# nzfeng/signed-heat-3d

Measured on AMD Instinct MI355X. Metric: grid-nodes/sec end-to-end SHM (conv+PCG), higher is better.
Workload: dtype f64 (Step 1: f64 / packed-f32 tiers)

## Files before the change

include/shm_grid.h:

```cpp
#ifndef SHM_GRID_H
#define SHM_GRID_H

#include <stddef.h>
#include <stdint.h>

#ifdef __cplusplus
extern "C" {
#endif

#define SHM_GRID_ABI_VERSION 5

typedef struct shm_solver shm_solver;

typedef enum {
    SHM_OK = 0,
    SHM_ERR_INVALID = 1,
    SHM_ERR_HIP = 2,
    SHM_ERR_NOMEM = 3,
    SHM_ERR_BREAKDOWN = 4,
    SHM_ERR_NOCONV = 5,
    SHM_ERR_RCCL = 6,
    SHM_ERR_STATE = 7,
    SHM_ERR_SINGULAR = 8
} shm_status;
// ... 24 lines not shown
    int32_t n;
    double bbox_min[3];
    double cell;
} shm_grid;

typedef struct {
    int32_t fast_integration;
    int32_t scrub_nonfinite;
    double tol;
    int32_t max_iters;
    int32_t check_every;
    int32_t preconditioner;
    int32_t solver;
    int32_t step1_arith;
    int32_t dual_form;
    double step1_budget;
} shm_opts;

enum { SHM_DUAL_AUTO = 0, SHM_DUAL_DIRECT = 1, SHM_DUAL_EXPLICIT_S_CG = 2, SHM_DUAL_THROUGH_GRID = 3 };

enum { SHM_STEP1_AUTO = 0, SHM_STEP1_EXACT_F64 = 1, SHM_STEP1_REFERENCE_F64 = 2 };

enum { SHM_SOLVER_AUTO = 0, SHM_SOLVER_PRIMAL = 1, SHM_SOLVER_DUAL = 2, SHM_SOLVER_DUAL_SLABS = 3 };

enum { SHM_PRECOND_AUTO = 0, SHM_PRECOND_NONE = 1, SHM_PRECOND_DCT = 2 };

typedef struct {
    int32_t n, m;
    int64_t S;
    int32_t iters;
    double rel_residual;
    double shift;
    double ms_conv;
    double ms_div;
    double ms_setup;
    double ms_wait_setup;
    double ms_pcg;
    double ms_shift;
    double ms_total;
    double ms_stencil_avg;
    double ms_update_xr_avg;
    double ms_project_avg;
    double ms_update_p_avg;
    double ms_precond_avg;
    int32_t kernel_samples;
    int32_t preconditioner;
    int32_t solver;
    double bytes_per_iter;
    int32_t cg_form;
    double pairs_fp64;
    double pairs_fp32;
    int32_t conv_launches;
    double pairs_redone;
} shm_stats;

shm_status shm_grid_create(const shm_config* cfg, shm_solver** out);
void shm_grid_destroy(shm_solver* s);
const char* shm_grid_last_error(const shm_solver* s);
int32_t shm_grid_abi_version(void);

shm_status shm_grid_set_problem(shm_solver* s, const shm_sources* src, const shm_grid* grid);
shm_status shm_grid_solve(shm_solver* s, const shm_opts* opts, shm_stats* stats);
shm_status shm_grid_get_phi(shm_solver* s, double* phi_out, int32_t* k_begin, int32_t* k_end);
shm_status shm_grid_owned_planes(shm_solver* s, int32_t* k_begin, int32_t* k_end);
shm_status shm_grid_compute_distance(shm_solver* s, const shm_sources* src, const shm_grid* grid,
                                     const shm_opts* opts, double* phi_out, shm_stats* stats);

typedef enum {
    SHM_FIELD_Y0 = 0,
    SHM_FIELD_Y1 = 1,
    SHM_FIELD_Y2 = 2,
    SHM_FIELD_DIV = 3,
    SHM_FIELD_PHI = 4
} shm_field;
shm_status shm_grid_run_conv(shm_solver* s);
shm_status shm_grid_run_conv_arith(shm_solver* s, int32_t step1_arith);
shm_status shm_grid_run_divergence(shm_solver* s, int32_t scrub);
shm_status shm_grid_get_field(shm_solver* s, shm_field f, double* out );
shm_status shm_grid_get_field_planes(shm_solver* s, shm_field f, int32_t k_begin, int32_t k_end, double* out);
shm_status shm_grid_apply_laplacian(shm_solver* s, const double* u, double* out);
shm_status shm_grid_set_phi(shm_solver* s, const double* phi );
shm_status shm_grid_get_constraints(shm_solver* s, int64_t* nodes, double* coeffs, int32_t* m);
shm_status shm_grid_get_schur(shm_solver* s, double* out, int32_t* m);
shm_status shm_grid_apply_projector(shm_solver* s, double* v);

shm_status shm_grid_apply_preconditioner(shm_solver* s, const double* v, double* out);

enum { SHM_ISO_MARCHING_CUBES = 0, SHM_ISO_MARCHING_TETS = 1 };
shm_status shm_grid_isosurface(shm_solver* s, double isovalue, int64_t* n_vertices, int64_t* n_triangles);
shm_status shm_grid_isosurface_ex(shm_solver* s, double isovalue, int32_t method, int64_t* n_vertices, int64_t* n_triangles);
shm_status shm_grid_get_isosurface(shm_solver* s, double* vertices , int64_t* triangles );

shm_status shm_grid_sample(shm_solver* s, int64_t Q, const double* pts, double* phi_out, double* grad_out, int64_t* n_answered);
shm_status shm_grid_sample_device(shm_solver* s, int64_t Q, const void* d_pts, void* d_phi, void* d_grad, int64_t* n_answered);

shm_status shm_grid_isosurface_indexed(shm_solver* s, double isovalue, int64_t* n_vertices, int64_t* n_triangles);
shm_status shm_grid_get_isosurface_indexed(shm_solver* s, double* vertices , int64_t* triangles );
shm_status shm_grid_get_isosurface_indexed_device(shm_solver* s, void* d_vertices , void* d_triangles );

typedef struct {
    int64_t first_vertex;
    int64_t n_vertices, n_triangles;
    double  area, volume;
    double  lo[3], hi[3];
    int32_t touches_box;
    int32_t reserved;
} shm_iso_component;
shm_status shm_grid_label_mesh_device(shm_solver* s, int64_t nv, int64_t nt, const void* d_triangles , void* d_root , int64_t* n_components);
shm_status shm_grid_isosurface_components(shm_solver* s, int64_t* n_components);
shm_status shm_grid_get_isosurface_components(shm_solver* s, shm_iso_component* comps , int64_t* tri_component ,
                                              int64_t* vertex_component );
shm_status shm_grid_isosurface_keep_components(shm_solver* s, const uint8_t* keep , int64_t* n_vertices, int64_t* n_triangles);

typedef struct {
    int64_t n_audited, n_not_owned, n_nonfinite, n_out_of_zone, n_finite_mismatch;
    double  max_dy;
    int64_t worst_node;
    double  worst_ratio;
    double  min_ratio;
    double  budget;
    int32_t step1_arith;
    int32_t within_budget;
    double  ms;
} shm_step1_audit;
shm_status shm_grid_audit_step1(shm_solver* s, int64_t count, const int64_t* nodes, double* dy_out , double* ratio_out ,
                                shm_step1_audit* out);
int64_t shm_audit_sample_nodes(int32_t n, int32_t k_begin, int32_t k_end, int64_t count, uint64_t seed, int64_t* nodes_out);

shm_status shm_grid_raycast(shm_solver* s, int64_t Q, const double* origins , const double* dirs , double isovalue, double t_min, double t_max,
                            double* t_out , double* grad_out , int64_t* n_hits);
shm_status shm_grid_raycast_device(shm_solver* s, int64_t Q, const void* d_origins, const void* d_dirs, double isovalue, double t_min, double t_max, void* d_t,
                                   void* d_grad, int64_t* n_hits);

typedef struct {
    int64_t n_frozen;
    int64_t n_reached;
    int64_t n_nonfinite;
    int64_t n_block_updates;
    int32_t n_rounds;
    int32_t reserved;
    double max_abs;
    double isovalue, band;
    double ms;
} shm_redistance_stats;
shm_status shm_grid_redistance(shm_solver* s, double isovalue, double band, shm_redistance_stats* out );
shm_status shm_grid_get_redistanced(shm_solver* s, double* psi_out );
shm_status shm_grid_get_redistanced_device(shm_solver* s, void* d_psi );

typedef struct {
    int64_t n_vertices, n_triangles;
    int64_t n_reached;
    int64_t n_candidate_pairs;
    double max_abs;
    double isovalue, band;
    double ms;
} shm_redistance_exact_stats;
shm_status shm_grid_redistance_exact(shm_solver* s, double isovalue, double band, shm_redistance_exact_stats* out );
shm_status shm_grid_isosurface_indexed_psi(shm_solver* s, double distance, int64_t* n_vertices, int64_t* n_triangles);

shm_status shm_grid_closest_point(shm_solver* s, int64_t Q, const double* pts , double max_dist, double* dist_out ,
                                  double* cp_out , int64_t* tri_out , int64_t* n_answered);
shm_status shm_grid_closest_point_device(shm_solver* s, int64_t Q, const void* d_pts, double max_dist, void* d_dist, void* d_cp ,
                                         void* d_tri , int64_t* n_answered);

shm_status shm_comm_unique_id(void* out128);
void shm_plan_slab(int32_t n, int32_t nslabs, int32_t slab, int32_t* k0, int32_t* k1);
// ... 8 lines not shown
```

signed-heat-3d_amd/csrc/shm_grid.hip:

```cpp
#include "shm_host.hip.h"
#include "shm_audit_sample.h"


struct shm_solver {
    std::unique_ptr<shm::SolverBase> impl;
    std::string err;
    shm_config cfg;
};

static thread_local std::string g_create_error;

template <typename F> static shm_status guard(shm_solver* s, F&& f) {
    if (!s) return SHM_ERR_INVALID;
    try {
        f();
        s->err.clear();
        return SHM_OK;
    } catch (const shm::Error& e) {
        s->err = e.what();
        return e.code;
    } catch (const std::bad_alloc&) {
        s->err = "host allocation failed";
        return SHM_ERR_NOMEM;
    } catch (const std::exception& e) {
// ... 82 lines not shown
    return guard(s, [&] {
        if (!src || !grid) throw shm::Error(SHM_ERR_INVALID, "null argument");
        s->impl->set_problem(*src, *grid);
    });
}

shm_status shm_grid_solve(shm_solver* s, const shm_opts* opts, shm_stats* stats) {
    return guard(s, [&] {
        shm_opts o;
        memset(&o, 0, sizeof o);
        o.scrub_nonfinite = 1;
        if (opts) o = *opts;
        s->impl->solve(o, stats);
    });
}

shm_status shm_grid_get_phi(shm_solver* s, double* phi_out, int32_t* k_begin, int32_t* k_end) {
    return guard(s, [&] {
        if (!phi_out) throw shm::Error(SHM_ERR_INVALID, "null phi_out");
        s->impl->get_phi(phi_out, k_begin, k_end);
    });
}

shm_status shm_grid_owned_planes(shm_solver* s, int32_t* k_begin, int32_t* k_end) {
    return guard(s, [&] { s->impl->owned_planes(k_begin, k_end); });
}

shm_status shm_grid_compute_distance(shm_solver* s, const shm_sources* src, const shm_grid* grid, const shm_opts* opts, double* phi_out,
                                     shm_stats* stats) {
    shm_status rc = shm_grid_set_problem(s, src, grid);
    if (rc != SHM_OK) return rc;
    if (s->cfg.world != 1) {
        s->err = "shm_grid_compute_distance is the single-process entry point; use set_problem/solve/get_phi per rank";
        return SHM_ERR_INVALID;
    }
    rc = shm_grid_solve(s, opts, stats);
    if (rc != SHM_OK && rc != SHM_ERR_NOCONV) return rc;
    std::string keep = s->err;
    shm_status rc2 = shm_grid_get_phi(s, phi_out, nullptr, nullptr);
    if (rc2 != SHM_OK) return rc2;
    s->err = keep;
    return rc;
}

shm_status shm_grid_run_conv(shm_solver* s) { return guard(s, [&] { s->impl->run_conv(SHM_STEP1_AUTO); }); }
shm_status shm_grid_run_conv_arith(shm_solver* s, int32_t step1_arith) { return guard(s, [&] { s->impl->run_conv(step1_arith); }); }
shm_status shm_grid_run_divergence(shm_solver* s, int32_t scrub) { return guard(s, [&] { s->impl->run_divergence(scrub); }); }
shm_status shm_grid_get_field(shm_solver* s, shm_field f, double* out) {
    return guard(s, [&] {
        if (!out) throw shm::Error(SHM_ERR_INVALID, "null out");
        s->impl->get_field(f, out);
    });
}
shm_status shm_grid_get_field_planes(shm_solver* s, shm_field f, int32_t k_begin, int32_t k_end, double* out) {
    return guard(s, [&] {
        if (!out) throw shm::Error(SHM_ERR_INVALID, "null out");
        s->impl->get_field_planes(f, k_begin, k_end, out);
    });
}
shm_status shm_grid_apply_laplacian(shm_solver* s, const double* u, double* out) {
    return guard(s, [&] {
        if (!u || !out) throw shm::Error(SHM_ERR_INVALID, "null argument");
        s->impl->apply_laplacian(u, out);
    });
}
shm_status shm_grid_set_phi(shm_solver* s, const double* phi) {
    return guard(s, [&] {
        if (!phi) throw shm::Error(SHM_ERR_INVALID, "null argument");
        s->impl->set_phi(phi);
    });
}
shm_status shm_grid_get_constraints(shm_solver* s, int64_t* nodes, double* coeffs, int32_t* m) {
    return guard(s, [&] {
        if (!nodes || !coeffs || !m) throw shm::Error(SHM_ERR_INVALID, "null argument");
        s->impl->get_constraints(nodes, coeffs, m);
    });
}
shm_status shm_grid_get_schur(shm_solver* s, double* out, int32_t* m) {
    return guard(s, [&] {
        if (!out || !m) throw shm::Error(SHM_ERR_INVALID, "null argument");
        s->impl->get_schur(out, m);
    });
}
shm_status shm_grid_apply_projector(shm_solver* s, double* v) {
    return guard(s, [&] {
        if (!v) throw shm::Error(SHM_ERR_INVALID, "null argument");
        s->impl->apply_projector(v);
    });
}

shm_status shm_grid_apply_preconditioner(shm_solver* s, const double* v, double* out) {
    return guard(s, [&] {
        if (!v || !out) throw shm::Error(SHM_ERR_INVALID, "null argument");
        s->impl->apply_preconditioner(v, out);
    });
}

shm_status shm_grid_isosurface(shm_solver* s, double isovalue, int64_t* n_vertices, int64_t* n_triangles) {
    return guard(s, [&] { s->impl->isosurface(isovalue, SHM_ISO_MARCHING_CUBES, n_vertices, n_triangles); });
}
shm_status shm_grid_isosurface_ex(shm_solver* s, double isovalue, int32_t method, int64_t* n_vertices, int64_t* n_triangles) {
    return guard(s, [&] { s->impl->isosurface(isovalue, method, n_vertices, n_triangles); });
}
shm_status shm_grid_get_isosurface(shm_solver* s, double* vertices, int64_t* triangles) {
    return guard(s, [&] { s->impl->get_isosurface(vertices, triangles); });
}

shm_status shm_grid_isosurface_indexed(shm_solver* s, double isovalue, int64_t* n_vertices, int64_t* n_triangles) {
    return guard(s, [&] { s->impl->isosurface_indexed(isovalue, n_vertices, n_triangles); });
}
shm_status shm_grid_get_isosurface_indexed(shm_solver* s, double* vertices, int64_t* triangles) {
    return guard(s, [&] { s->impl->get_isosurface_indexed(vertices, triangles); });
}
shm_status shm_grid_get_isosurface_indexed_device(shm_solver* s, void* d_vertices, void* d_triangles) {
    return guard(s, [&] { s->impl->get_isosurface_indexed_device(d_vertices, d_triangles); });
}

shm_status shm_grid_label_mesh_device(shm_solver* s, int64_t nv, int64_t nt, const void* d_triangles, void* d_root, int64_t* n_components) {
    return guard(s, [&] { s->impl->label_mesh_device(nv, nt, d_triangles, d_root, n_components); });
}
shm_status shm_grid_isosurface_components(shm_solver* s, int64_t* n_components) {
    return guard(s, [&] { s->impl->isosurface_components(n_components); });
}
shm_status shm_grid_get_isosurface_components(shm_solver* s, shm_iso_component* comps, int64_t* tri_component, int64_t* vertex_component) {
    return guard(s, [&] { s->impl->get_isosurface_components(comps, tri_component, vertex_component); });
}
shm_status shm_grid_isosurface_keep_components(shm_solver* s, const uint8_t* keep, int64_t* n_vertices, int64_t* n_triangles) {
    return guard(s, [&] { s->impl->isosurface_keep_components(keep, n_vertices, n_triangles); });
}

shm_status shm_grid_sample(shm_solver* s, int64_t Q, const double* pts, double* phi_out, double* grad_out, int64_t* n_answered) {
    return guard(s, [&] { s->impl->sample(Q, pts, phi_out, grad_out, n_answered); });
}
shm_status shm_grid_sample_device(shm_solver* s, int64_t Q, const void* d_pts, void* d_phi, void* d_grad, int64_t* n_answered) {
    return guard(s, [&] { s->impl->sample_device(Q, d_pts, d_phi, d_grad, n_answered); });
}

shm_status shm_grid_raycast(shm_solver* s, int64_t Q, const double* origins, const double* dirs, double isovalue, double t_min, double t_max, double* t_out,
                            double* grad_out, int64_t* n_hits) {
    return guard(s, [&] { s->impl->raycast(Q, origins, dirs, isovalue, t_min, t_max, t_out, grad_out, n_hits); });
}
shm_status shm_grid_raycast_device(shm_solver* s, int64_t Q, const void* d_origins, const void* d_dirs, double isovalue, double t_min, double t_max, void* d_t,
                                   void* d_grad, int64_t* n_hits) {
    return guard(s, [&] { s->impl->raycast_device(Q, d_origins, d_dirs, isovalue, t_min, t_max, d_t, d_grad, n_hits); });
}

shm_status shm_grid_redistance(shm_solver* s, double isovalue, double band, shm_redistance_stats* out) {
    return guard(s, [&] { s->impl->redistance(isovalue, band, out); });
}
shm_status shm_grid_redistance_exact(shm_solver* s, double isovalue, double band, shm_redistance_exact_stats* out) {
    return guard(s, [&] { s->impl->redistance_exact(isovalue, band, out); });
}
shm_status shm_grid_isosurface_indexed_psi(shm_solver* s, double distance, int64_t* n_vertices, int64_t* n_triangles) {
    return guard(s, [&] { s->impl->isosurface_indexed_psi(distance, n_vertices, n_triangles); });
}
shm_status shm_grid_get_redistanced(shm_solver* s, double* psi_out) {
    return guard(s, [&] { s->impl->get_redistanced(psi_out); });
}
shm_status shm_grid_get_redistanced_device(shm_solver* s, void* d_psi) {
    return guard(s, [&] { s->impl->get_redistanced_device(d_psi); });
}

shm_status shm_grid_closest_point(shm_solver* s, int64_t Q, const double* pts, double max_dist, double* dist_out, double* cp_out, int64_t* tri_out, int64_t* n_answered) {
    return guard(s, [&] { s->impl->closest_point(Q, pts, max_dist, dist_out, cp_out, tri_out, n_answered); });
}
shm_status shm_grid_closest_point_device(shm_solver* s, int64_t Q, const void* d_pts, double max_dist, void* d_dist, void* d_cp, void* d_tri, int64_t* n_answered) {
// ... 30 lines not shown
```

signed-heat-3d_amd/csrc/shm_host.hip.h:

```cpp
#pragma once
#include <hip/hip_runtime.h>
#include <rccl/rccl.h>

#include <dlfcn.h>

#include <algorithm>
#include <atomic>
#include <chrono>
#include <cmath>
#include <cstdarg>
#include <cstdio>
#include <cstring>
#include <limits>
#include <memory>
#include <mutex>
#include <stdexcept>
#include <string>
#include <thread>
#include <unordered_map>
#include <unordered_set>
#include <vector>

#include "../../include/shm_grid.h"
#include "shm_constraints.h"
// ... 409 lines not shown
                            lbs[(size_t)(s - g0)] = rel - lhs_drop;
                            if (lbs[(size_t)(s - g0)] <= ln_tau) {
                                bnd[(size_t)(s - g0)] = std::exp(lbs[(size_t)(s - g0)]) * r_hi / d_box;
                                gsum += bnd[(size_t)(s - g0)];
                            }
                        }
                        const bool soft_ok = R + gsum <= eps_soft;
                        if (soft_ok) R += gsum;
                        for (int64_t s = g0; s < g1; s++) {
                            if (!(wmag[(size_t)s] > 0.)) continue;
                            if (bnd[(size_t)(s - g0)] >= 0. && (soft_ok || lbs[(size_t)(s - g0)] <= ln_tau_hard)) continue;
                            const double lhs = lambda * (dist[(size_t)s] - rt - r_hi), rel = std::log(wmag[(size_t)s]) - ln_near;
                            const double d_box = std::max(0., dist[(size_t)s] - rt), d0 = std::max(0., dmin - rt);
                            const bool in_range = 1.4426950408889634 * lambda * (d_box - d0) + range_c <= std::log2(wmag[(size_t)s]) - lwhi;
                            cost += lhs > tier_log + rel && in_range ? far_cost : 1.0;
                        }
                    }
                } else {
                    for (size_t c = 0; c < crad.size(); c++) {
                        const double dx = cx - ccen[3 * c], dy = cy - ccen[3 * c + 1], dz = cz - ccen[3 * c + 2];
                        const double gap = std::sqrt(dx * dx + dy * dy + dz * dz) - rt - crad[c] - r_hi;
                        if (!(gap * lambda > skip_base + clnw[c] - ln_near)) cost += kCl;
                    }
                }
                acc += cost;
            }
        const double per_plane = acc / ((double)K * K * (double)S) + 1e-3;
        for (int k = L * bz; k < std::min(n, (L + 1) * bz); k++) weights[k] = per_plane;
    };
    const unsigned hw = std::thread::hardware_concurrency();
    const int nthr = (int)std::max(1u, std::min({hw ? hw : 1u, 16u, (unsigned)layers, (unsigned)(((double)layers * K * K * (double)S) / 2e6 + 1.)}));
    std::atomic<int> next{0};
    auto worker = [&]() {
        std::vector<double> dist((size_t)S);
        for (int L = next.fetch_add(1); L < layers; L = next.fetch_add(1)) do_layer(L, dist);
    };
    std::vector<std::thread> pool;
    for (int t = 1; t < nthr; t++) pool.emplace_back(worker);
    worker();
    for (std::thread& t : pool) t.join();
}

static void plan_slabs_weighted(int n, int nslabs, const double* w, int granule, std::vector<int32_t>& bounds) {
    bounds.assign((size_t)nslabs + 1, 0);
    bounds[(size_t)nslabs] = n;
    if (granule < 1) granule = 1;
    if ((long long)granule * nslabs > n) granule = std::max(1, n / nslabs);
    std::vector<double> cum((size_t)n + 1, 0.);
    for (int k = 0; k < n; k++) cum[(size_t)k + 1] = cum[(size_t)k] + (w && w[k] > 0. ? w[k] : 0.);
    if (!(cum[(size_t)n] > 0.))
        for (int k = 0; k <= n; k++) cum[(size_t)k] = k;
    for (int i = 1; i < nslabs; i++) {
        const double target = cum[(size_t)n] * i / nslabs;
        const int lo = bounds[(size_t)i - 1] + granule, hi = n - (nslabs - i) * granule;
        int best = lo;
        double best_err = 1e300;
        for (int k = ((lo + granule - 1) / granule) * granule; k <= hi; k += granule) {
            const double e = std::fabs(cum[(size_t)k] - target);
            if (e < best_err) {
                best_err = e;
                best = k;
            }
        }
        bounds[(size_t)i] = std::min(std::max(best, lo), std::max(lo, hi));
    }
}

struct SolverBase {
    virtual ~SolverBase() = default;
    virtual void set_problem(const shm_sources&, const shm_grid&) = 0;
    virtual void solve(const shm_opts&, shm_stats*) = 0;
    virtual void get_phi(double*, int32_t*, int32_t*) = 0;
    virtual void owned_planes(int32_t*, int32_t*) = 0;
    virtual void run_conv(int step1_arith) = 0;
    virtual void run_divergence(int scrub) = 0;
    virtual void get_field(shm_field, double*) = 0;
    virtual void get_field_planes(shm_field, int, int, double*) = 0;
    virtual void apply_laplacian(const double*, double*) = 0;
    virtual void set_phi(const double*) = 0;
    virtual void get_constraints(int64_t*, double*, int32_t*) = 0;
    virtual void apply_projector(double*) = 0;
    virtual void apply_preconditioner(const double*, double*) = 0;
    virtual void get_schur(double*, int32_t*) = 0;
    virtual void isosurface(double, int, int64_t*, int64_t*) = 0;
    virtual void get_isosurface(double*, int64_t*) = 0;
    virtual void sample(int64_t, const double*, double*, double*, int64_t*) = 0;
    virtual void sample_device(int64_t, const void*, void*, void*, int64_t*) = 0;
    virtual void isosurface_indexed(double, int64_t*, int64_t*) = 0;
    virtual void get_isosurface_indexed(double*, int64_t*) = 0;
    virtual void get_isosurface_indexed_device(void*, void*) = 0;
    virtual void label_mesh_device(int64_t, int64_t, const void*, void*, int64_t*) = 0;
    virtual void isosurface_components(int64_t*) = 0;
    virtual void get_isosurface_components(shm_iso_component*, int64_t*, int64_t*) = 0;
    virtual void isosurface_keep_components(const uint8_t*, int64_t*, int64_t*) = 0;
    virtual void audit_step1(int64_t, const int64_t*, double*, double*, shm_step1_audit*) = 0;
    virtual void raycast(int64_t, const double*, const double*, double, double, double, double*, double*, int64_t*) = 0;
    virtual void raycast_device(int64_t, const void*, const void*, double, double, double, void*, void*, int64_t*) = 0;
    virtual void redistance(double, double, shm_redistance_stats*) = 0;
    virtual void get_redistanced(double*) = 0;
    virtual void get_redistanced_device(void*) = 0;
    virtual void redistance_exact(double, double, shm_redistance_exact_stats*) = 0;
    virtual void isosurface_indexed_psi(double, int64_t*, int64_t*) = 0;
    virtual void closest_point(int64_t, const double*, double, double*, double*, int64_t*, int64_t*) = 0;
    virtual void closest_point_device(int64_t, const void*, double, void*, void*, void*, int64_t*) = 0;
};

SolverBase* make_solver_f64(const shm_config& cfg);
SolverBase* make_solver_f32(const shm_config& cfg);

}
```

signed-heat-3d_amd/csrc/shm_kernels.hip.h:

```cpp
#pragma once
#include <hip/hip_runtime.h>
#include <stdint.h>

#include <type_traits>

#include "shm_constraints.h"
#include "shm_mc_table.h"

namespace shm {

constexpr int kBlock = 256;
constexpr int kMaxPartials = 8192;

__device__ __forceinline__ double wave_sum(double v) {
#pragma unroll
    for (int off = 32; off > 0; off >>= 1) v += __shfl_down(v, off, kWave);
    return v;
}

__device__ __forceinline__ double block_sum(double v, double* lds ) {
    v = wave_sum(v);
    const int lane = threadIdx.x & 63, w = threadIdx.x >> 6;
    if (lane == 0) lds[w] = v;
    __syncthreads();
    double s = 0.;
    if (threadIdx.x == 0) {
        const int nw = (blockDim.x * blockDim.y + 63) >> 6;
        for (int a = 0; a < nw; a++) s += lds[a];
    }
    return s;
}

__device__ __forceinline__ unsigned xcd_remap(unsigned bid, unsigned nblk) {
    const unsigned xcd = bid & 7u, slot = bid >> 3;
    const unsigned q = nblk >> 3, r = nblk & 7u;
    const unsigned base = (xcd < r) ? xcd * (q + 1) : r * (q + 1) + (xcd - r) * q;
    return base + slot;
}

constexpr int kSrcTile = 256;

template <typename T> struct YukawaMath;
template <> struct YukawaMath<double> {
    static constexpr int kExpTabBits = 11;
    static __device__ __forceinline__ double yukawa(double x, double c, const double* __restrict__ tab ) {
        const double y0 = __builtin_amdgcn_rsq(x);
        const double t = x * y0;
        const double e = fma(-t, y0, 1.0);
        const double q = fma(e, 0.375, 0.5) * e;
        const double r = fma(t, q, t);
        const double rinv = fma(y0, q, y0);
        const double tm = fma(r, c, 6755399441055744.0);
        const double kf = tm - 6755399441055744.0;
        const int ki = (int)(unsigned)__double_as_longlong(tm);
        const double f = fma(r, c, -kf);
        double p = 6.461528672932366e-12;
        p = fma(p, f, 5.727446245172041e-08);
        p = fma(p, f, 3.384507717577858e-04);
        p = fma(p, f, 1.0);
        return __builtin_amdgcn_ldexp(tab[ki & ((1 << kExpTabBits) - 1)] * p * rinv, ki >> kExpTabBits);
    }
    static __device__ __forceinline__ double exp_neg(double x) {
        const double kf = rint(x * 1.4426950408889634074);
        double f = fma(kf, -6.93147180369123816490e-01, x);
        f = fma(kf, -1.90821492927058770002e-10, f);
        double p = 1.6059043836821613e-10;
        p = fma(p, f, 2.08767569878681e-09);
        p = fma(p, f, 2.505210838544172e-08);
        p = fma(p, f, 2.755731922398589e-07);
        p = fma(p, f, 2.7557319223985893e-06);
        p = fma(p, f, 2.48015873015873e-05);
        p = fma(p, f, 1.984126984126984e-04);
        p = fma(p, f, 1.3888888888888889e-03);
        p = fma(p, f, 8.333333333333333e-03);
        p = fma(p, f, 4.1666666666666664e-02);
        p = fma(p, f, 1.6666666666666666e-01);
        p = fma(p, f, 0.5);
        p = fma(p, f, 1.0);
        p = fma(p, f, 1.0);
        return __builtin_amdgcn_ldexp(p, (int)kf);
    }
};
template <> struct YukawaMath<float> {
    static __device__ __forceinline__ void rsqrt_and_sqrt(float x, float& rinv, float& r) {
        const float y0 = __builtin_amdgcn_rsqf(x);
        r = x * y0;
        rinv = y0;
    }
    static __device__ __forceinline__ float exp_neg(float x) { return __expf(x); }
// ... 1394 lines not shown
            const int j = t & (kGJ - 1), k2 = t >> 6;
            rs[k2][j] = R[(size_t)(r_row0 + kc + k2) * ld + oj + j];
        }
        __syncthreads();
#pragma unroll
        for (int kk = 0; kk < kGJK; kk += 4) {
            double af[2], bf[2];
#pragma unroll
            for (int a = 0; a < 2; a++) af[a] = cs[wr * 32 + a * 16 + l15][kk + l4];
#pragma unroll
            for (int b = 0; b < 2; b++) bf[b] = rs[kk + l4][wc * 32 + b * 16 + l15];
#pragma unroll
            for (int a = 0; a < 2; a++)
#pragma unroll
                for (int b = 0; b < 2; b++) acc[a][b] = __builtin_amdgcn_mfma_f64_16x16x4f64(af[a], bf[b], acc[a][b], 0, 0, 0);
        }
    }
    const bool prow = kb >= 0 && bi == kb, pcol = kb >= 0 && bj == kb;
    const size_t o = (size_t)kb * kGJ;
#pragma unroll
    for (int a = 0; a < 2; a++)
#pragma unroll
        for (int b = 0; b < 2; b++)
#pragma unroll
            for (int r = 0; r < 4; r++) {
                const size_t row = oi + wr * 32 + a * 16 + l4 + 4 * r, col = oj + wc * 32 + b * 16 + l15;
                double* dst = &G[row * ld + col];
                const double v = acc[a][b][r];
                if (prow) *dst = R[(size_t)(r_row0 + (int)(row - o)) * ld + col];
                else if (pcol) *dst = -v;
                else *dst -= v;
            }
}
template <int TILES>
__global__ __launch_bounds__(kBlock) void gj_update_kernel(double* __restrict__ G_, int ld, int nb, int kb ,
                                                           int k0, int nO, const double* __restrict__ R_ , int r_row0,
                                                           const double* __restrict__ C_ , int c_ld, int c_col0, int K, int prio,
                                                           GjBatch Bt = GjBatch{nullptr, nullptr, nullptr, nullptr, nullptr, nullptr, nullptr}) {
    __shared__ double smem[kGjUpdateLds];
    if (prio) __builtin_amdgcn_s_setprio(3);
    double* G = G_;
    const double* R = R_;
    const double* C = C_;
    if (Bt.D) {
        const int a = blockIdx.y;
        ld = gj_batch_ld(Bt, a);
        nb = ld / kGJ;
        if (kb >= nb || blockIdx.x >= (unsigned)(nb * (nb + 1) / 2)) return;
        G = Bt.D + Bt.offD[a];
        R = Bt.R + Bt.offW[a];
        C = Bt.C + Bt.offW[a];
        c_ld = kGJ;
    }
    int bi, bj;
    if (TILES == GJ_ALL) {
        gj_tri_decode(blockIdx.x, bi, bj);
    } else if (TILES == GJ_CROSS) {
        const int idx = (int)blockIdx.x;
        if (idx < nO * nb) {
            bj = k0 + idx % nO;
            bi = idx / nO;
            if (bi < bj) return;
        } else {
            const int r = idx - nO * nb;
            bi = k0 + r % nO;
            bj = r / nO;
        }
    } else {
        gj_tri_decode(blockIdx.x, bi, bj);
        if (bi >= k0) bi += nO;
        if (bj >= k0) bj += nO;
    }
    gj_update_tile(G, ld, bi, bj, TILES != GJ_REST ? kb : -1, R, r_row0, C, c_ld, c_col0, K, smem);
}

#ifndef SHM_GJ_STEP_PAIRS
#define SHM_GJ_STEP_PAIRS 1
#endif
#ifndef SHM_GJ_STEP_WAVES
#define SHM_GJ_STEP_WAVES 3
#endif
constexpr int kGjStepScratch = 8 * (kGJ + 1);
constexpr int kGjStepLds = kGJ * (kGJ + 1) + kGjStepScratch;
static __global__ __launch_bounds__(kBlock) __attribute__((amdgpu_waves_per_eu(SHM_GJ_STEP_WAVES, SHM_GJ_STEP_WAVES))) void gj_step_kernel(
    double* __restrict__ G, int ld, int nb, int k, const double* __restrict__ Rp , const double* __restrict__ Cp ,
    double* __restrict__ Rn, double* __restrict__ Cn, int* __restrict__ flag, int prio) {
    __shared__ double smem[kGjStepLds];
    static_assert(kGjStepLds >= kGjUpdateLds && kGjStepScratch >= 8 * kGJ, "LDS carve");
    if (prio) __builtin_amdgcn_s_setprio(3);
    const int nN = k < nb ? nb : 0;
    if ((int)blockIdx.x >= nN) {
        int bi, bj;
        gj_tri_decode(blockIdx.x - (unsigned)nN, bi, bj);
        if (k < nb) {
            if (bi >= k) bi += 1;
            if (bj >= k) bj += 1;
        }
        gj_update_tile(G, ld, bi, bj, k - 1, Rp, 0, Cp, kGJ, 0, kGJ, smem);
        return;
    }
    double(*x)[kGJ + 1] = reinterpret_cast<double(*)[kGJ + 1]>(smem);
    double* scratch = smem + kGJ * (kGJ + 1);
    double(*prow)[kGJ + 1] = reinterpret_cast<double(*)[kGJ + 1]>(scratch);
    const int b = blockIdx.x;
    const bool below = b >= k;
    const int bi = below ? b : k, bj = below ? k : b;
    const size_t o = (size_t)k * kGJ, ob = (size_t)b * kGJ, oi = (size_t)bi * kGJ, oj = (size_t)bj * kGJ;
    const int lane = threadIdx.x & 63, w = threadIdx.x >> 6, wr = w >> 1, wc = w & 1, l15 = lane & 15, l4 = lane >> 4;
    const int ty = threadIdx.x >> 4, tx = threadIdx.x & 15;
    double r[4][4];
    double* Cb = Cn + ob * kGJ;
    if (k > 0) {
        auto product = [&](gj_f64x4(&acc)[2][2], size_t orow, size_t ocol) {
#pragma unroll
            for (int a = 0; a < 2; a++)
#pragma unroll
                for (int c = 0; c < 2; c++) acc[a][c] = gj_f64x4{0., 0., 0., 0.};
#pragma unroll 1
            for (int g = 0; g < 2; g++) {
                double af[8][2], bf[8][2];
#pragma unroll
                for (int u = 0; u < 8; u++) {
                    const int kk = 32 * g + 4 * u + l4;
#pragma unroll
                    for (int a = 0; a < 2; a++) af[u][a] = Cp[(orow + wr * 32 + a * 16 + l15) * kGJ + kk];
#pragma unroll
                    for (int c = 0; c < 2; c++) bf[u][c] = Rp[(size_t)kk * ld + ocol + wc * 32 + c * 16 + l15];
                }
#pragma unroll
                for (int u = 0; u < 8; u++)
#pragma unroll
                    for (int a = 0; a < 2; a++)
#pragma unroll
                        for (int c = 0; c < 2; c++) acc[a][c] = __builtin_amdgcn_mfma_f64_16x16x4f64(af[u][a], bf[u][c], acc[a][c], 0, 0, 0);
            }
        };
        {
            gj_f64x4 accp[2][2];
            product(accp, o, o);
#pragma unroll
            for (int a = 0; a < 2; a++)
#pragma unroll
                for (int c = 0; c < 2; c++)
#pragma unroll
                    for (int q = 0; q < 4; q++) {
                        const size_t row = wr * 32 + a * 16 + l4 + 4 * q, col = wc * 32 + c * 16 + l15;
                        x[row][col] = G[(o + row) * ld + o + col] - accp[a][c][q];
                    }
        }
        gj_f64x4 accx[2][2];
        product(accx, oi, oj);
        __syncthreads();
#pragma unroll
        for (int a = 0; a < 4; a++)
#pragma unroll
            for (int c = 0; c < 4; c++) r[a][c] = x[ty * 4 + a][tx * 4 + c];
        __syncthreads();
        const double keep = b == k - 1 ? 0. : 1.;
#pragma unroll
        for (int a = 0; a < 2; a++)
#pragma unroll
            for (int c = 0; c < 2; c++)
#pragma unroll
                for (int q = 0; q < 4; q++) {
                    const size_t row = wr * 32 + a * 16 + l4 + 4 * q, col = wc * 32 + c * 16 + l15;
                    x[row][col] = G[(oi + row) * ld + oj + col] * keep - accx[a][c][q];
                }
    } else {
        for (int t = threadIdx.x; t < kGJ * kGJ; t += kBlock) {
            const int i = t / kGJ, j = t % kGJ;
            x[i][j] = G[(oi + i) * ld + oj + j];
        }
#pragma unroll
        for (int a = 0; a < 4; a++)
#pragma unroll
            for (int c = 0; c < 4; c++) r[a][c] = G[(o + ty * 4 + a) * ld + o + tx * 4 + c];
    }
    __syncthreads();
    for (int t = threadIdx.x; t < kGJ * kGJ; t += kBlock) {
        const int i = t / kGJ, j = t % kGJ;
        Cb[i * kGJ + j] = below ? x[i][j] : -x[j][i];
    }
    gj_invert64_scalar<4, SHM_GJ_STEP_PAIRS != 0>(r, scratch, flag);
    if (b == k) {
#pragma unroll
        for (int a = 0; a < 4; a++)
#pragma unroll
            for (int c = 0; c < 4; c++) Rn[(size_t)(ty * 4 + a) * ld + ob + tx * 4 + c] = r[a][c];
        return;
    }
    double pa[2][kGJ / 4];
#pragma unroll
    for (int pass = 0; pass < 8; pass++) {
        __syncthreads();
        if ((ty >> 1) == pass) {
#pragma unroll
            for (int a = 0; a < 4; a++)
#pragma unroll
                for (int c = 0; c < 4; c++) prow[(ty & 1) * 4 + a][tx * 4 + c] = r[a][c];
        }
        __syncthreads();
        if (wr == (pass >> 2) && (l15 >> 3) == (pass & 1)) {
#pragma unroll
            for (int s4 = 0; s4 < kGJ / 4; s4++) pa[(pass >> 1) & 1][s4] = prow[l15 & 7][4 * s4 + l4];
        }
    }
    gj_f64x4 acc[2][2];
#pragma unroll
    for (int a = 0; a < 2; a++)
#pragma unroll
        for (int c = 0; c < 2; c++) acc[a][c] = gj_f64x4{0., 0., 0., 0.};
#pragma unroll
    for (int s4 = 0; s4 < kGJ / 4; s4++) {
        const int kk = 4 * s4 + l4;
        double bf[2];
#pragma unroll
        for (int c = 0; c < 2; c++) {
            const int j = wc * 32 + c * 16 + l15;
            bf[c] = (b > k) ? x[j][kk] : x[kk][j];
        }
#pragma unroll
        for (int a = 0; a < 2; a++)
#pragma unroll
            for (int c = 0; c < 2; c++) acc[a][c] = __builtin_amdgcn_mfma_f64_16x16x4f64(pa[a][s4], bf[c], acc[a][c], 0, 0, 0);
    }
#pragma unroll
    for (int a = 0; a < 2; a++)
#pragma unroll
        for (int c = 0; c < 2; c++)
#pragma unroll
            for (int q = 0; q < 4; q++) Rn[(size_t)(wr * 32 + a * 16 + l4 + 4 * q) * ld + ob + wc * 32 + c * 16 + l15] = acc[a][c][q];
}

static __global__ __launch_bounds__(kBlock) void gj_mirror_kernel(double* __restrict__ G_, int ld, GjBatch Bt = GjBatch{nullptr, nullptr, nullptr, nullptr, nullptr, nullptr, nullptr}) {
    __shared__ double x[kGJ][kGJ + 1];
    double* G = G_;
    if (Bt.D) {
        const int a = blockIdx.y;
        ld = gj_batch_ld(Bt, a);
        const int nb = ld / kGJ;
        if (blockIdx.x >= (unsigned)(nb * (nb - 1) / 2)) return;
        G = Bt.D + Bt.offD[a];
    }
    const unsigned t = blockIdx.x;
    int bi = (int)((sqrt(8.0 * (double)t + 1.0) - 1.0) * 0.5);
    while ((unsigned)bi * (unsigned)(bi + 1) / 2 > t) bi--;
    while ((unsigned)(bi + 1) * (unsigned)(bi + 2) / 2 <= t) bi++;
    const int bj = (int)(t - (unsigned)bi * (unsigned)(bi + 1) / 2);
    bi += 1;
    const size_t oi = (size_t)bi * kGJ, oj = (size_t)bj * kGJ;
    for (int e = threadIdx.x; e < kGJ * kGJ; e += kBlock) {
        const int i = e / kGJ, j = e % kGJ;
        x[i][j] = G[(oi + i) * ld + oj + j];
    }
    __syncthreads();
    for (int e = threadIdx.x; e < kGJ * kGJ; e += kBlock) {
        const int i = e / kGJ, j = e % kGJ;
        G[(oj + i) * ld + oi + j] = x[j][i];
    }
}

struct IsoParams {
    int n, nzl, k0;
    double bbox_min[3];
    double cell;
    double iso;
};

__device__ __constant__ int kKuhnTets[6][4] = {{0, 1, 3, 7}, {0, 1, 5, 7}, {0, 2, 3, 7}, {0, 2, 6, 7}, {0, 4, 5, 7}, {0, 4, 6, 7}};

__device__ __forceinline__ int tet_tris(int mask) {
    const int c = __popc(mask);
    return c == 0 || c == 4 ? 0 : (c == 2 ? 2 : 1);
}

template <typename T, bool EMIT>
__global__ __launch_bounds__(kBlock) void iso_kernel(IsoParams P, const T* __restrict__ phi , unsigned long long* __restrict__ counter,
                                                     double* __restrict__ tri_pos , unsigned long long* __restrict__ tri_keys ,
                                                     unsigned long long* __restrict__ tri_sort , unsigned long long cap) {
    __shared__ double red[8];
    const int n = P.n, nc = n - 1;
    const size_t plane = (size_t)n * n;
    const int kend = min(P.nzl, n - 1 - P.k0);
    const size_t ncells = (size_t)nc * nc * (size_t)max(kend, 0);
    double mycount = 0.;
    for (size_t c = (size_t)blockIdx.x * kBlock + threadIdx.x; c < ncells; c += (size_t)gridDim.x * kBlock) {
        const int kk = (int)(c / ((size_t)nc * nc));
        const int rem = (int)(c - (size_t)kk * nc * nc);
        const int j = rem / nc, i = rem - j * nc;
        const size_t base = (size_t)(kk + 1) * plane + (size_t)j * n + i;
        double v[8];
        int inside = 0;
        bool fin = true;
#pragma unroll
        for (int q = 0; q < 8; q++) {
            v[q] = (double)phi[base + (q & 1) + ((q >> 1) & 1) * (size_t)n + ((q >> 2) & 1) * plane];
            inside |= (v[q] < P.iso ? 1 : 0) << q;
            fin &= v[q] - v[q] == 0.;
        }
        if (inside == 0 || inside == 255 || !fin) continue;
        const int k = P.k0 + kk;
        const unsigned long long gnode = (unsigned long long)i + (unsigned long long)j * n + (unsigned long long)k * plane;
        for (int t = 0; t < 6; t++) {
            int tv[4], mask = 0;
#pragma unroll
            for (int a = 0; a < 4; a++) {
                tv[a] = kKuhnTets[t][a];
                mask |= ((inside >> tv[a]) & 1) << a;
            }
            const int nt = tet_tris(mask);
            if (nt == 0) continue;
            if (!EMIT) {
                mycount += nt;
                continue;
// ... 128 lines not shown
```

signed-heat-3d_amd/csrc/shm_plan.h:

```cpp
#pragma once
#include <algorithm>
#include <cmath>
#include <cstdint>
#include <cstdlib>

#include "../../include/shm_grid.h"

namespace shm {

enum Step1Kernel { kStep1TieredF64, kStep1TieredF32, kStep1Untiered };
enum PlanPath { kPathFast, kPathGathered, kPathDualSlabs, kPathDualLocal, kPathPrimalFused, kPathPrimalClassic };

struct PlanKnobs {
    bool no_direct = false;
    bool no_dense_s = false;
    bool dense_s_always = false;
    int tl_min_m = 6144;
};
template <typename Get> PlanKnobs plan_knobs(Get knob) {
    PlanKnobs k;
    k.no_direct = knob("SHM_DUAL_NO_DIRECT") != nullptr;
    k.no_dense_s = knob("SHM_DUAL_NO_DENSE_S") != nullptr;
    k.dense_s_always = knob("SHM_DUAL_DENSE_S_ALWAYS") != nullptr;
    if (knob("SHM_TL_MIN_M")) k.tl_min_m = atoi(knob("SHM_TL_MIN_M"));
    return k;
}

struct PlanIn {
    bool f64 = true;
    int n = 0;
    int64_t S = 0;
    int total_slabs = 1;
    bool full_wanted = false, fft_available = false, gemm_dct = false, fused_available = false;
    Step1Kernel step1 = kStep1Untiered;
    double conv_est_total_ms = 1e30;
    int solver = SHM_SOLVER_AUTO, preconditioner = SHM_PRECOND_AUTO, dual_form = SHM_DUAL_AUTO;
    double step1_budget = 0.;
    bool fast = false;
    PlanKnobs knobs;
    bool precond_available() const { return fft_available || gemm_dct; }
    bool tiered() const { return step1 != kStep1Untiered; }
};

struct Plan {
    shm_status status = SHM_OK;
    const char* error = nullptr;
    PlanPath path = kPathPrimalClassic;
    bool precond = false;
    bool dual_requested = false;
    int setup_prio = 1;
    bool green_early = false;
    int dual_form = SHM_DUAL_THROUGH_GRID;
    bool explicit_S = false;
    bool two_level = false;
    double est_setup_ms = -1., est_step1_ms = -1.;
};

inline Plan plan_error(shm_status s, const char* msg) { Plan p; p.status = s; p.error = msg; return p; }

inline Plan plan_solve(const PlanIn& in) {
    Plan p;
    if (in.preconditioner == SHM_PRECOND_DCT) {
        if (!in.precond_available())
            return plan_error(SHM_ERR_INVALID, "DCT preconditioner needs n = 2^k in [16,1024] and a power-of-two number of EQUAL z-slabs dividing n (shm_config.slab_plan = SHM_SLAB_PLAN_EQUAL); a single z-slab serves any n in [4,1024]");
        p.precond = true;
    } else if (in.preconditioner == SHM_PRECOND_AUTO) {
        p.precond = in.precond_available();
    } else if (in.preconditioner != SHM_PRECOND_NONE) {
        return plan_error(SHM_ERR_INVALID, "unknown preconditioner");
    }
    if (in.dual_form < SHM_DUAL_AUTO || in.dual_form > SHM_DUAL_THROUGH_GRID) return plan_error(SHM_ERR_INVALID, "unknown dual_form");
    if (in.step1_budget != 0. && !(in.step1_budget >= 1e-12 && in.step1_budget <= 1e-3)) return plan_error(SHM_ERR_INVALID, "step1_budget must lie in [1e-12, 1e-3] (0: default 1e-8)");
    if (in.solver != SHM_SOLVER_AUTO && in.solver != SHM_SOLVER_PRIMAL && in.solver != SHM_SOLVER_DUAL && in.solver != SHM_SOLVER_DUAL_SLABS)
        return plan_error(SHM_ERR_INVALID, "unknown solver");
    if (in.fast) {
        p.path = kPathFast;
        return p;
    }
    const bool with_precond = in.preconditioner != SHM_PRECOND_NONE;
    const bool slab_forms_auto = in.solver == SHM_SOLVER_AUTO && with_precond && in.fft_available && in.total_slabs >= 4 && in.n >= 256 && in.n <= 512 && in.S <= 16384 &&
                                 in.dual_form != SHM_DUAL_THROUGH_GRID;
    if (in.full_wanted && !slab_forms_auto && (in.solver == SHM_SOLVER_AUTO || in.solver == SHM_SOLVER_DUAL) && with_precond) {
        p.path = kPathGathered;
        return p;
    }
    p.dual_requested = (in.solver == SHM_SOLVER_DUAL || in.solver == SHM_SOLVER_DUAL_SLABS || (in.solver == SHM_SOLVER_AUTO && with_precond)) && in.precond_available();
    bool dual = false;
    if (in.solver == SHM_SOLVER_DUAL || in.solver == SHM_SOLVER_DUAL_SLABS) {
        if (!in.precond_available())
            return plan_error(SHM_ERR_INVALID, "the dual solver needs the DCT: n = 2^k in [16,1024] and a power-of-two number of EQUAL z-slabs dividing n (shm_config.slab_plan = SHM_SLAB_PLAN_EQUAL); a single z-slab serves any n in [4,1024]");
        dual = true;
    } else if (in.solver == SHM_SOLVER_AUTO) {
        dual = in.precond_available() && with_precond;
    }
    if (dual) p.path = in.total_slabs > 1 ? kPathDualSlabs : kPathDualLocal;
    else p.path = in.fused_available ? kPathPrimalFused : kPathPrimalClassic;
    return p;
}

inline void plan_setup(const PlanIn& in, Plan& p) {
    p.setup_prio = in.step1 == kStep1TieredF64 && in.conv_est_total_ms >= 150. && in.conv_est_total_ms < 1e29 ? 0 : 1;
    const bool iterative_form = in.dual_form == SHM_DUAL_EXPLICIT_S_CG || in.dual_form == SHM_DUAL_THROUGH_GRID;
    p.green_early = !iterative_form && p.dual_requested && !in.knobs.no_direct && !in.knobs.no_dense_s && (in.total_slabs == 1 || in.fft_available) &&
                    in.precond_available() && !in.gemm_dct && in.n <= 512 && in.S > 0 && in.S <= 4096 &&
                    (in.f64 || in.step1 == kStep1TieredF32 || in.n < 512 || in.dual_form == SHM_DUAL_DIRECT);
}

inline bool plan_explicit_S(const PlanIn& in, int m, bool direct) {
    const bool off = in.knobs.no_dense_s || in.dual_form == SHM_DUAL_THROUGH_GRID;
    if (in.gemm_dct) return !off && m > 0 && m <= 16384;
    if (in.total_slabs > 1) return !off && in.fft_available && m > 0 && m <= 16384 && in.n <= 512;
    const bool asked = in.dual_form == SHM_DUAL_DIRECT || in.dual_form == SHM_DUAL_EXPLICIT_S_CG;
    const int max_m = (in.tiered() || asked) ? 16384 : 8192;
    if (off || !in.precond_available() || m <= 0 || m > max_m || in.n > 512) return false;
    if (in.knobs.dense_s_always || asked || direct) return true;
    const double md = (double)m, width = in.f64 ? 1.0 : 0.5;
    const double schur_est_ms = 2.2e-7 * md * md;
    const double dense_iter_ms = 3.6e-9 * md * md * width + 0.08;
    const double grid_iter_ms = std::max(0.15, 1.4 * std::pow((double)in.n / 512.0, 3.0) * width);
    return in.tiered() && in.conv_est_total_ms >= 3.0 * schur_est_ms && grid_iter_ms > 1.3 * dense_iter_ms;
}

template <typename Est> void plan_rows(const PlanIn& in, int m, Est step1_ms, Plan& p) {
    const bool no_direct = in.knobs.no_direct || in.dual_form == SHM_DUAL_EXPLICIT_S_CG || in.dual_form == SHM_DUAL_THROUGH_GRID;
    const int direct_max_m = in.dual_form == SHM_DUAL_DIRECT ? 16384 : 4096;
    bool direct = p.dual_requested && !no_direct && m <= direct_max_m;
    if (!direct && p.dual_requested && !no_direct && in.tiered() && in.precond_available() && !in.gemm_dct && in.n <= 512 && m > direct_max_m && m <= 16384 &&
        in.conv_est_total_ms < 1e29) {
        const double md = (double)m;
        p.est_setup_ms = 5.5e-11 * md * md * md + 1.4e-7 * md * md + 10.0 * std::pow((double)in.n / 512.0, 4.0);
        p.est_step1_ms = step1_ms();
        direct = p.est_setup_ms <= 0.38 * p.est_step1_ms;
    }
    if (!in.f64 && in.step1 != kStep1TieredF32 && in.n >= 512 && !in.gemm_dct && in.dual_form != SHM_DUAL_DIRECT) direct = false;
    direct = direct && plan_explicit_S(in, m, true);
    p.explicit_S = plan_explicit_S(in, m, direct);
    p.dual_form = direct ? SHM_DUAL_DIRECT : p.explicit_S ? SHM_DUAL_EXPLICIT_S_CG : SHM_DUAL_THROUGH_GRID;
    p.two_level = !direct && m > in.knobs.tl_min_m;
}

inline const char* plan_path_name(PlanPath path) {
    static const char* const names[] = {"fast", "gathered", "dual-slabs", "dual", "primal-fused", "primal-classic"};
    return names[path];
}

}
```

signed-heat-3d_amd/csrc/shm_solver.hip.h:

```cpp
#pragma once
#include "shm_host.hip.h"
#include "shm_kernels.hip.h"
#include "shm_conv_tiered.hip.h"
#include "shm_cg_fused.hip.h"
#include "shm_twolevel.hip.h"
#include "shm_schur.hip.h"
#include "shm_dct.hip.h"
#include "shm_dct_gemm.hip.h"
#include "shm_green_fft.hip.h"
#include "shm_sample.hip.h"
#include "shm_audit.hip.h"
#include "shm_iso_indexed.hip.h"
#include "shm_iso_components.hip.h"
#include "shm_raycast.hip.h"
#include "shm_redistance.hip.h"
#include "shm_redistance_exact.hip.h"
#include "shm_closest.hip.h"
#include "shm_plan.h"

namespace shm {

template <typename T> constexpr int vec_width() { return sizeof(T) == 8 ? 2 : 4; }

template <typename T>
// ... 44 lines not shown
    double conv_ctr[3] = {0, 0, 0};
    double conv_wscale = 1.;
    int64_t S = 0;
    std::vector<double> h_pos, h_wn, h_area;
    double area_sum = 0., conv_far_gap = 0., conv_skip_base = 3.0e38, last_host_setup_ms = 0., last_setup_wall_ms = 0.;
    double conv_tier_ring = 0.;
    double conv_tier_log = 0., conv_tier_skip_base = 3.0e38;
    double conv_drop_K = 64., conv_drop_eps64 = 2e-9, conv_drop_eps32 = 6.0e-8;
    double conv_w_span = 0.;
    DevArray<double> d_src_t;
    DevArray<float> d_clusters_t;
    int n_clusters_t = 0;
    bool conv_tiered = false;
    bool conv_tier_exact = false;
    bool conv_tiered32 = false;
    bool conv_reference = false;
    int step1_selected = SHM_STEP1_AUTO;
    int last_step1_arith = SHM_STEP1_AUTO;
    double last_step1_budget = 0.;
    bool fold_pq = false;
    int fold_pq_np = 0;
    double step1_budget = 0.;
    DevArray<unsigned long long> d_pair_counters;
    DevArray<unsigned> d_unit_counters;
    static constexpr int kMaxConvLaunches = 256;
    int conv_launch_index = 0;
    int conv_launches_last = 0;
    int n_clusters = 0;
    int conv_grid_cap = 1 << 30;
    bool o_fast_hint = false;
    int num_cus = 256;
    DevArray<T> d_src;
    DevArray<float> d_src32;
    DevArray<float> d_clusters;
    DevArray<double> d_exptab;
    std::vector<Slab<T>> slabs;
    int total_slabs = 1, first_slab = 0;
    std::vector<int32_t> slab_bounds;
    bool slabs_equal = true;
    void slab_range(int slab, int32_t* k0, int32_t* k1) const {
        *k0 = slab_bounds[(size_t)slab];
        *k1 = slab_bounds[(size_t)slab + 1];
    }
    bool have_problem = false, have_conv = false, have_div = false, have_phi = false, have_constraints = false;
    std::vector<Row> rows;
    std::vector<std::vector<ShiftItem>> shift_host;
    int m = 0, mp = 0;
    DevArray<double> Ginv, gjP, gjR, gjC;
    DevArray<float> Ginv32;
    struct TwoLevel {
        bool on = false;
        int box = 16, P = 0, nI = 0, nS = 0, nSp = 0, ysz = 0;
        DevArray<int> ptrI, ptrS, rowsI, colsS, sepRow, adj_ptr, adj_idx, colour_list, rowBox, chunkBox, chunkCol, tBox, tRow, sBox, sRow;
        DevArray<size_t> offW;
        DevArray<double> gjP, gjR, gjC;
        int nChunks = 0, nTChunks = 0, nbMax = 0;
        int schur_ptr[9] = {0, 0, 0, 0, 0, 0, 0, 0, 0};
        DevArray<size_t> offD, offE;
        DevArray<double> D, E, Tm, tbuf, ybuf, vS, uS;
        DevArray<float> D32, E32, T32;
        int colour_ptr[9] = {0, 0, 0, 0, 0, 0, 0, 0, 0};
        size_t szD = 0, szE = 0;
        TlBoxes view() const { return TlBoxes{ptrI.p, ptrS.p, offD.p, offE.p, rowsI.p, colsS.p}; }
    } tl;
    int ginv_rows = 0, ginv_ld = 0;
    DevArray<int> gjFlag;
    DevArray<double*> d_redptrs;
    DevArray<int> Bptr, Bcol;
    DevArray<double> Bval;
    bool have_B = false;
    using TP = T;
    DevArray<Cplx<TP>> d_tw, d_om;
    DevArray<TP> d_lam;
    DevArray<double> d_lam64;
    DevArray<double> gd_Cm, gd_Ct, gd_W1, gd_W2;
    DevArray<double> gs_lam, gs_ctab, gs_Cm, gs_Ct, gs_W0, gs_W1, gs_T, Sdense, d_rowT;
    DevArray<int> d_rowX;
    std::vector<double> h_gs_lam, h_gs_ctab, h_rowT;
    std::vector<Cplx<double>> h_gs_tw;
    DevArray<Cplx<double>> gs_tw;
    std::vector<int> h_rowX;
    bool have_S = false;
    DevArray<double> Sinv, Sinv_ones ;
    PlanIn plan_in;
    Plan plan;
    double conv_est_total_ms = 1e30;
    int log2n = 0;
    bool precond_ready = false;
    double* h_pinned = nullptr;
    Rccl::comm_t comm = nullptr;
    int vec = 1;
    std::unique_ptr<Solver<T>> full;
    bool solve_only = false;
    bool full_problem_set = false;
    bool pool_held = false;

    explicit Solver(const shm_config& c, bool solve_only_ = false) : cfg(c), solve_only(solve_only_) {
        int ndev = 0;
        hipError_t e = hipGetDeviceCount(&ndev);
        if (e != hipSuccess || ndev <= 0)
            throw Error(SHM_ERR_HIP, fmt("no HIP device available (%s); this library has no CPU fallback",
                                          e == hipSuccess ? "device count 0" : hipGetErrorString(e)));
        if (cfg.device < 0 || cfg.device >= ndev) throw Error(SHM_ERR_INVALID, fmt("device %d out of range [0,%d)", cfg.device, ndev));
        HIPCHK(hipSetDevice(cfg.device));
        HIPCHK(hipStreamCreateWithFlags(&stream, hipStreamNonBlocking));
        {
            hipDeviceProp_t prop;
            HIPCHK(hipGetDeviceProperties(&prop, cfg.device));
            conv_grid_cap = std::max(1, prop.multiProcessorCount * 4);
            num_cus = prop.multiProcessorCount;
        }
        {
            int least = 0, greatest = 0;
            HIPCHK(hipDeviceGetStreamPriorityRange(&least, &greatest));
            HIPCHK(hipStreamCreateWithPriority(&stream2, hipStreamNonBlocking, greatest));
        }
        HIPCHK(hipHostMalloc((void**)&h_pinned, 64 * sizeof(double)));
        if (cfg.world > 1 && !cfg.rccl_unique_id) throw Error(SHM_ERR_INVALID, "world>1 needs rccl_unique_id");
        if (cfg.rccl_unique_id) {
            Rccl& R = Rccl::get();
            Rccl::unique_id id;
            memcpy(&id, cfg.rccl_unique_id, sizeof id);
            R.chk(R.CommInitRank(&comm, cfg.world, id, cfg.rank), "ncclCommInitRank");
        }
        PinnedPool::get().acquire(cfg.device);
        pool_held = true;
    }
    ~Solver() override {
        (void)hipSetDevice(cfg.device);
        if (comm) (void)Rccl::get().CommDestroy(comm);
        if (h_pinned) (void)hipHostFree(h_pinned);
        for (void* b : smp_pinned)
            if (b) (void)hipHostFree(b);
        for (void* b : ray_pinned)
            if (b) (void)hipHostFree(b);
        slabs.clear();
        if (stream) (void)hipStreamDestroy(stream);
        if (stream2) (void)hipStreamDestroy(stream2);
        if (stream3) (void)hipStreamDestroy(stream3);
        if (stream_h) (void)hipStreamDestroy(stream_h);
        if (pool_held) PinnedPool::get().release(cfg.device);
    }

    void log(const char* f, ...) {
        if (!cfg.verbose) return;
        va_list ap;
        va_start(ap, f);
        vfprintf(stderr, f, ap);
        va_end(ap);
        fputc('\n', stderr);
    }

    static int grid_for(size_t work_items, int cap = 2048) {
        size_t b = (work_items + kBlock - 1) / kBlock;
        if (b < 1) b = 1;
        if (b > (size_t)cap) b = cap;
        return (int)b;
    }

    void set_problem(const shm_sources& src, const shm_grid& g) override {
        HIPCHK(hipSetDevice(cfg.device));
        if (g.n < 2) throw Error(SHM_ERR_INVALID, "grid.n must be >= 2");
        if (!(g.cell > 0.) || !std::isfinite(g.cell)) throw Error(SHM_ERR_INVALID, "grid.cell must be positive and finite");
        if (src.S <= 0 || !src.pos || !src.wnormal || !src.area) throw Error(SHM_ERR_INVALID, "sources: S>0 and non-null arrays required");
        if (!(src.lambda > 0.) || !std::isfinite(src.lambda)) throw Error(SHM_ERR_INVALID, "sources.lambda must be positive and finite");
        if (src.S > (int64_t)1 << 28) throw Error(SHM_ERR_INVALID, "too many sources");
// ... 889 lines not shown
        HIPCHK(hipGetLastError());
        log("[shm] two-level inverse of A A^T: box %d, %d boxes (%d interior rows, largest box %d rows x %d separator columns), separator %d rows", tl.box, P, tl.nI, part.maxs, part.maxc, tl.nS);
        return true;
    }

    void apply_Ginv(const double* w, double* u, bool f32, hipStream_t st) {
        if (m <= 0) return;
        if (!tl.on) {
            if (f32) launch_ginv_matvec<float>(st, m, m, mp, Ginv32.p, w, u);
            else launch_ginv_matvec<double>(st, m, m, mp, Ginv.p, w, u);
            return;
        }
        const TlBoxes V = tl.view();
        const unsigned grows = (unsigned)((tl.nI + kBlock / kWave - 1) / (kBlock / kWave));
        if (f32) hipLaunchKernelGGL((tl_rows_kernel<float>), dim3(grows), dim3(kBlock), 0, st, V, tl.rowBox.p, tl.nI, tl.D32.p, w, tl.tbuf.p);
        else hipLaunchKernelGGL((tl_rows_kernel<double>), dim3(grows), dim3(kBlock), 0, st, V, tl.rowBox.p, tl.nI, tl.D.p, w, tl.tbuf.p);
        if (tl.nChunks > 0) {
            if (f32) hipLaunchKernelGGL((tl_cols_kernel<float>), dim3((unsigned)tl.nChunks), dim3(kBlock), 0, st, V, tl.chunkBox.p, tl.chunkCol.p, tl.E32.p, tl.tbuf.p, tl.ybuf.p);
            else hipLaunchKernelGGL((tl_cols_kernel<double>), dim3((unsigned)tl.nChunks), dim3(kBlock), 0, st, V, tl.chunkBox.p, tl.chunkCol.p, tl.E.p, tl.tbuf.p, tl.ybuf.p);
        }
        hipLaunchKernelGGL(tl_gather_sep_kernel, dim3((unsigned)((tl.nS + kBlock - 1) / kBlock)), dim3(kBlock), 0, st, tl.nS, tl.sepRow.p, tl.adj_ptr.p, tl.adj_idx.p, w,
                           tl.ybuf.p, tl.vS.p);
        if (f32) launch_ginv_matvec<float>(st, tl.nS, tl.nS, tl.nSp, Ginv32.p, tl.vS.p, tl.uS.p);
        else launch_ginv_matvec<double>(st, tl.nS, tl.nS, tl.nSp, Ginv.p, tl.vS.p, tl.uS.p);
        const unsigned gfin = grows + (unsigned)((tl.nS + kBlock - 1) / kBlock);
        if (f32) hipLaunchKernelGGL((tl_finish_kernel<float>), dim3(gfin), dim3(kBlock), 0, st, V, tl.rowBox.p, tl.nI, tl.nS, tl.sepRow.p, tl.T32.p, tl.tbuf.p, tl.uS.p, u);
        else hipLaunchKernelGGL((tl_finish_kernel<double>), dim3(gfin), dim3(kBlock), 0, st, V, tl.rowBox.p, tl.nI, tl.nS, tl.sepRow.p, tl.Tm.p, tl.tbuf.p, tl.uS.p, u);
    }

    void enqueue_gj_invert(double* M, int mp, bool refined_later = false) {
        hipStream_t stream = stream2;
        const int nb = mp / kGJ;
        const int outer = nb >= 64 ? 4 : 1;
        gjP.alloc(kGJ * kGJ);
        gjR.alloc((size_t)outer * kGJ * mp);
        gjC.alloc((size_t)mp * outer * kGJ);
        gjFlag.alloc(2);
        HIPCHK(hipMemsetAsync(gjFlag.p, 0, sizeof(int), stream));
        const int c_ld = outer * kGJ;
        const bool classic = knob("SHM_GJ_CLASSIC") != nullptr;
        const bool stepped = outer == 1 && !classic;
        auto launch_pivot = [&](int kb) {
            if (refined_later) hipLaunchKernelGGL(gj_pivot_block4_kernel, dim3(1), dim3(256), 0, stream, M, mp, kb, gjP.p, gjFlag.p, plan.setup_prio);
            else hipLaunchKernelGGL(gj_pivot_kernel<4>, dim3(1), dim3(256), 0, stream, M, mp, kb, gjP.p, gjFlag.p, plan.setup_prio);
        };
        if (stepped) {
            gjR.alloc((size_t)2 * kGJ * mp);
            gjC.alloc((size_t)2 * mp * kGJ);
            for (int k = 0; k <= nb; k++) {
                const size_t nU = k == 0 ? 0 : (k < nb ? (size_t)(nb - 1) * nb / 2 : (size_t)nb * (nb + 1) / 2);
                const unsigned grid = (unsigned)((k < nb ? nb : 0) + nU);
                double* Rn = gjR.p + (size_t)(k & 1) * kGJ * mp;
                double* Cn = gjC.p + (size_t)(k & 1) * mp * kGJ;
                const double* Rp = gjR.p + (size_t)((k + 1) & 1) * kGJ * mp;
                const double* Cp = gjC.p + (size_t)((k + 1) & 1) * mp * kGJ;
                hipLaunchKernelGGL(gj_step_kernel, dim3(grid), dim3(kBlock), 0, stream, M, mp, nb, k, Rp, Cp, Rn, Cn, gjFlag.p, plan.setup_prio);
            }
        } else if (outer == 1) {
            for (int kb = 0; kb < nb; kb++) {
                launch_pivot(kb);
                hipLaunchKernelGGL(gj_panels_kernel, dim3(nb), dim3(kBlock), 0, stream, M, mp, kb, gjP.p, gjR.p, 0, gjC.p, c_ld, 0, plan.setup_prio);
                hipLaunchKernelGGL((gj_update_kernel<GJ_ALL>), dim3((unsigned)((size_t)nb * (nb + 1) / 2)), dim3(kBlock), 0, stream, M, mp, nb, kb, 0, 1,
                                   gjR.p, 0, gjC.p, c_ld, 0, kGJ, plan.setup_prio);
            }
        } else {
            for (int k0 = 0; k0 < nb; k0 += outer) {
                const int nO = std::min(outer, nb - k0);
                for (int t = 0; t < nO; t++) {
                    const int kb = k0 + t;
                    launch_pivot(kb);
                    hipLaunchKernelGGL(gj_panels_kernel, dim3(nb), dim3(kBlock), 0, stream, M, mp, kb, gjP.p, gjR.p, t * kGJ, gjC.p, c_ld, t * kGJ, plan.setup_prio);
                    hipLaunchKernelGGL((gj_update_kernel<GJ_CROSS>), dim3((unsigned)(nO * nb + nO * k0)), dim3(kBlock), 0, stream, M, mp, nb, kb, k0, nO,
                                       gjR.p, t * kGJ, gjC.p, c_ld, t * kGJ, kGJ, plan.setup_prio);
                }
                const size_t nr = (size_t)(nb - nO);
                if (nr > 0)
                    hipLaunchKernelGGL((gj_update_kernel<GJ_REST>), dim3((unsigned)(nr * (nr + 1) / 2)), dim3(kBlock), 0, stream, M, mp, nb, -1, k0, nO,
                                       gjR.p, 0, gjC.p, c_ld, 0, nO * kGJ, plan.setup_prio);
            }
        }
        if (nb > 1) hipLaunchKernelGGL(gj_mirror_kernel, dim3((unsigned)((size_t)nb * (nb - 1) / 2)), dim3(kBlock), 0, stream, M, mp);
        HIPCHK(hipGetLastError());
    }
    void enqueue_invert_G() {
        const int mp = ginv_ld;
        enqueue_gj_invert(Ginv.p, mp);
        Ginv32.alloc((size_t)mp * mp);
        hipLaunchKernelGGL((convert_kernel<double, float>), dim3(grid_for((size_t)mp * mp, 4096)), dim3(kBlock), 0, stream2, (size_t)mp * mp, Ginv.p, Ginv32.p);
        HIPCHK(hipGetLastError());
    }
    void enqueue_green_table(hipStream_t st) {
        const int P = n + 8;
        const size_t n1 = (size_t)n + 1;
        {
            const double pi = 3.14159265358979323846;
            h_gs_lam.resize(n);
            h_gs_ctab.resize(2 * (size_t)n);
            for (int k = 0; k < n; k++) h_gs_lam[k] = (2. - 2. * std::cos(pi * k / n)) / (cell * cell);
            for (int r = 0; r < 2 * n; r++) h_gs_ctab[r] = std::cos(pi * r / n);
            gs_lam.upload(h_gs_lam, st);
            gs_ctab.upload(h_gs_ctab, st);
            gs_T.alloc(n1 * n1 * P);
        }
        {
            DevArray<double>&W0 = gs_W0, &W1 = gs_W1, &W2 = gs_W0;
            gs_Cm.alloc(n1 * n);
            gs_Ct.alloc((size_t)n * P);
            W0.alloc(std::max((size_t)n * n * n, (size_t)n * n1 * P));
            W1.alloc((size_t)n * n * P);
            const bool by_fft = (n & (n - 1)) == 0 && n >= 16 && n <= 512;
            if (by_fft) {
                const double pi = 3.14159265358979323846;
                h_gs_tw.resize(2 * (size_t)n);
                for (int t = 0; t < n; t++) {
                    h_gs_tw[(size_t)t] = {std::cos(2. * pi * t / n), -std::sin(2. * pi * t / n)};
                    h_gs_tw[(size_t)n + t] = {std::cos(pi * t / n), -std::sin(pi * t / n)};
                }
                gs_tw.upload(h_gs_tw, st);
                HIPCHK(hipMemsetAsync(W1.p, 0, (size_t)n * n * P * sizeof(double), st));
                hipLaunchKernelGGL(green_symbol_kernel, dim3((unsigned)std::min(n * n, 8 * num_cus)), dim3(kBlock), 0, st, n, gs_lam.p, W0.p);
                const long long Pl = P, n1l = (long long)n1;
                auto pass = [&](bool xpass, int ntiles, int tiles_a, DctAddr in, DctAddr out, const double* src, double* dst) {
                    CosiParams C;
                    C.ntiles = ntiles;
                    C.tiles_a = tiles_a;
                    C.in = in;
                    C.out = out;
                    const dim3 g((unsigned)std::min(ntiles, 16 * num_cus));
                    const Cplx<double>*tw = gs_tw.p, *om = gs_tw.p + n;
                    int l2 = 0;
                    while ((1 << l2) < n) l2++;
#define SHM_COSI_CASE(L)                                                                                                                              \
    case L:                                                                                                                                            \
        if (xpass) hipLaunchKernelGGL((cosi_lines_kernel<L, true>), g, dim3(kBlock), 0, st, C, src, dst, tw, om, plan.setup_prio);                         \
        else hipLaunchKernelGGL((cosi_lines_kernel<L, false>), g, dim3(kBlock), 0, st, C, src, dst, tw, om, plan.setup_prio);                              \
        break;
                    switch (l2) {
                        SHM_COSI_CASE(4) SHM_COSI_CASE(5) SHM_COSI_CASE(6) SHM_COSI_CASE(7) SHM_COSI_CASE(8) SHM_COSI_CASE(9)
                        default: throw Error(SHM_ERR_INVALID, "Green's table by FFT: n out of range");
                    }
#undef SHM_COSI_CASE
                };
                auto addr = [](long long a_stride, long long b_stride, long long line_stride, long long elem_stride) {
                    DctAddr A;
                    A.off = 0; A.a_stride = a_stride; A.b_stride = b_stride; A.line_stride = line_stride; A.elem_stride = elem_stride;
                    A.seg_stride = 0; A.seg_shift = 30; A.seg_mask = 0x3fffffff;
                    return A;
                };
                const int L = kCosiL;
                pass(true, n * n / L, n * n / L, addr((long long)L * n, 0, n, 1), addr((long long)L * Pl, 0, Pl, 1), W0.p, W1.p);
                pass(false, n * (P / L), P / L, addr(L, (long long)n * Pl, 1, Pl), addr(L, n1l * Pl, 1, Pl), W1.p, W2.p);
                pass(false, (int)(n1l * Pl / L), (int)(n1l * Pl / L), addr(L, 0, 1, n1l * Pl), addr(L, 0, 1, n1l * Pl), W2.p, gs_T.p);
                HIPCHK(hipGetLastError());
                return;
            }
            HIPCHK(hipMemsetAsync(gs_Ct.p, 0, (size_t)n * P * sizeof(double), st));
            hipLaunchKernelGGL(cosine_tables_kernel, dim3(grid_for(n1 * n, 1024)), dim3(kBlock), 0, st, n, P, gs_ctab.p, gs_Cm.p, gs_Ct.p);
            hipLaunchKernelGGL(green_symbol_kernel, dim3((unsigned)std::min(n * n, 8 * num_cus)), dim3(kBlock), 0, st, n, gs_lam.p, W0.p);
            const bool narrow = plan_in.tiered();
            auto tiles = [](size_t v) { return (unsigned)((v + kGemmT - 1) / kGemmT); };
            auto gemm = [&](unsigned batches, int M, int N, int K, const double* A, int lda, long long sA, const double* B, int ldb, long long sB, double* C, int ldc, long long sC) {
                if (narrow)
                    hipLaunchKernelGGL(dgemm_rm_kernel<1>, dim3((unsigned)((N + 31) / 32), tiles((size_t)M), batches), dim3(kBlock), 0, st, M, N, K, A, lda, sA, B, ldb, sB, C, ldc, sC, plan.setup_prio);
                else
                    hipLaunchKernelGGL(dgemm_rm_kernel<4>, dim3(tiles((size_t)N), tiles((size_t)M), batches), dim3(kBlock), 0, st, M, N, K, A, lda, sA, B, ldb, sB, C, ldc, sC, plan.setup_prio);
            };
            gemm(1, n * n, P, n, W0.p, n, 0LL, gs_Ct.p, P, 0LL, W1.p, P, 0LL);
            gemm((unsigned)n, (int)n1, P, n, gs_Cm.p, n, 0LL, W1.p, P, (long long)n * P, W2.p, P, (long long)(n1 * P));
            gemm(1, (int)n1, (int)(n1 * P), n, gs_Cm.p, n, 0LL, W2.p, (int)(n1 * P), 0LL, gs_T.p, (int)(n1 * P), 0LL);
            HIPCHK(hipGetLastError());
        }
    }
    void prepare_schur() {
        hipStream_t st = stream2;
        have_S = false;
        if (!plan.explicit_S) return;
        if (!plan.green_early) enqueue_green_table(st);
        schur_row_order(rows, h_rowX, h_rowT);
        d_rowX.upload(h_rowX, st);
        d_rowT.upload(h_rowT, st);
        Sdense.alloc((size_t)mp * mp);
        if (!stream3) {
            int least = 0, greatest = 0;
            HIPCHK(hipDeviceGetStreamPriorityRange(&least, &greatest));
            HIPCHK(hipStreamCreateWithPriority(&stream3, hipStreamNonBlocking, greatest));
            e_sch_in.reset(new Event());
            e_sch_done.reset(new Event());
        }
        e_sch_in->record(st);
    }
    void enqueue_schur() {
        if (!plan.explicit_S) return;
        const bool dual_direct = plan.dual_form == SHM_DUAL_DIRECT;
        hipStream_t st = dual_direct ? stream2 : stream3;
        HIPCHK(hipStreamWaitEvent(st, e_sch_in->e, 0));
        const int P = n + 8;
        if (plan.green_early) HIPCHK(hipStreamWaitEvent(st, e_gs_done->e, 0));
        HIPCHK(hipMemsetAsync(Sdense.p, 0, (size_t)mp * mp * sizeof(double), st));
        const unsigned mt = (unsigned)((m + 15) / 16);
        hipLaunchKernelGGL(schur_assemble_kernel, dim3(mt, mt), dim3(kBlock), 0, st, m, mp, n, P, d_rowX.p, d_rowT.p, gs_T.p, Sdense.p, plan.setup_prio);
        HIPCHK(hipGetLastError());
        if (dual_direct) {
            Sinv.alloc((size_t)mp * mp);
            HIPCHK(hipMemcpyAsync(Sinv.p, Sdense.p, (size_t)mp * mp * sizeof(double), hipMemcpyDeviceToDevice, st));
            if (mp > m) hipLaunchKernelGGL(set_diagonal_kernel, dim3((unsigned)((mp - m + kBlock - 1) / kBlock)), dim3(kBlock), 0, st, Sinv.p, mp, m, mp, 1.0);
            enqueue_gj_invert(Sinv.p, mp, true);
            Sinv_ones.alloc((size_t)2 * mp);
            hipLaunchKernelGGL(fill_kernel, dim3((unsigned)((m + kBlock - 1) / kBlock)), dim3(kBlock), 0, st, Sinv_ones.p + mp, m, 1.0);
            launch_ginv_matvec<double>(st, m, m, mp, Sinv.p, Sinv_ones.p + mp, Sinv_ones.p);
        } else {
            e_sch_done->record(st);
            HIPCHK(hipStreamWaitEvent(stream2, e_sch_done->e, 0));
        }
        have_S = true;
    }
    void finish_invert_G() {
        hipStream_t stream = stream2;
        int flag[2] = {0, 0};
        if (!tl.on) HIPCHK(hipMemsetAsync(gjFlag.p + 1, 0, sizeof(int), stream));
        HIPCHK(hipMemcpyAsync(flag, gjFlag.p, 2 * sizeof(int), hipMemcpyDeviceToHost, stream));
        HIPCHK(hipStreamSynchronize(stream));
        if (flag[0] || flag[1]) throw Error(SHM_ERR_SINGULAR, "A A^T is not positive definite (duplicate or degenerate constraint rows)");
    }

    void allreduce(int which , int count) {
        auto buf = [&](Slab<T>& sl) { return which == 0 ? sl.red.p : sl.pq.p; };
        if (slabs.size() > 1) {
            double** slot = d_redptrs.p + (which ? slabs.size() : 0);
            hipLaunchKernelGGL(sum_slabs_kernel, dim3((count + kBlock - 1) / kBlock), dim3(kBlock), 0, stream, (int)slabs.size(), slot, count);
        }
        if (comm) {
            Rccl& R = Rccl::get();
            R.chk(R.AllReduce(buf(slabs[0]), buf(slabs[0]), (size_t)count, Rccl::kFloat64, Rccl::kSum, comm, stream), "ncclAllReduce");
            for (size_t s = 1; s < slabs.size(); s++)
                HIPCHK(hipMemcpyAsync(buf(slabs[s]), buf(slabs[0]), (size_t)count * sizeof(double), hipMemcpyDeviceToDevice, stream));
        }
    }

    void halo_exchange_p() { halo_exchange(ARR_P); }
    void halo_exchange(int sel) { halo_exchange(sel, stream); }
    void halo_exchange(int sel, hipStream_t stream) {
        const size_t pb = slabs[0].plane * sizeof(T);
        for (size_t s = 0; s + 1 < slabs.size(); s++) {
            Slab<T>&a = slabs[s], &b = slabs[s + 1];
            HIPCHK(hipMemcpyAsync(arr(b, sel), arr(a, sel) + (size_t)a.nzl * a.plane, pb, hipMemcpyDeviceToDevice, stream));
            HIPCHK(hipMemcpyAsync(arr(a, sel) + (size_t)(a.nzl + 1) * a.plane, arr(b, sel) + b.plane, pb, hipMemcpyDeviceToDevice, stream));
        }
        if (comm) {
            Rccl& R = Rccl::get();
            const int dt = sizeof(T) == 8 ? Rccl::kFloat64 : Rccl::kFloat32;
            Slab<T>&lo = slabs.front(), &hi = slabs.back();
            const size_t cnt = lo.plane;
            R.chk(R.GroupStart(), "ncclGroupStart");
            if (cfg.rank > 0) {
                R.chk(R.Send(arr(lo, sel) + lo.plane, cnt, dt, cfg.rank - 1, comm, stream), "ncclSend(lo)");
                R.chk(R.Recv(arr(lo, sel), cnt, dt, cfg.rank - 1, comm, stream), "ncclRecv(lo)");
            }
            if (cfg.rank < cfg.world - 1) {
                R.chk(R.Send(arr(hi, sel) + (size_t)hi.nzl * hi.plane, cnt, dt, cfg.rank + 1, comm, stream), "ncclSend(hi)");
                R.chk(R.Recv(arr(hi, sel) + (size_t)(hi.nzl + 1) * hi.plane, cnt, dt, cfg.rank + 1, comm, stream), "ncclRecv(hi)");
            }
            R.chk(R.GroupEnd(), "ncclGroupEnd");
        }
    }

    struct StencilLaunch {
        dim3 grid, block;
        int xchunks, yblocks, zc;
    };
    StencilLaunch stencil_dims(const Slab<T>& sl) const {
        const int per_row = (n + vec - 1) / vec;
        int tx = 1;
        while (tx < per_row && tx < kBlock) tx <<= 1;
        const int tyb = kBlock / tx;
        const int xchunks = (per_row + tx - 1) / tx;
        const int yblocks = (n + tyb * kStRY - 1) / (tyb * kStRY);
        int zc = 16;
        while (zc > 4 && (long long)xchunks * yblocks * ((sl.nzl + zc - 1) / zc) < 1024) zc >>= 1;
        const int zchunks = (sl.nzl + zc - 1) / zc;
        return {dim3((unsigned)(xchunks * yblocks * zchunks)), dim3((unsigned)tx, (unsigned)tyb), xchunks, yblocks, zc};
    }

    void launch_stencil(Slab<T>& sl) {
        const StencilLaunch L = stencil_dims(sl);
        if (vec == 1)
            hipLaunchKernelGGL((stencil_dot_kernel<T, 1>), L.grid, L.block, 0, stream, sl.gp, L.xchunks, L.yblocks, L.zc, sl.p.p, sl.q.p, sl.partials.p);
        else
            hipLaunchKernelGGL((stencil_dot_kernel<T, vec_width<T>()>), L.grid, L.block, 0, stream, sl.gp, L.xchunks, L.yblocks, L.zc, sl.p.p, sl.q.p, sl.partials.p);
    }

    template <int VEC> void launch_update_xr(Slab<T>& sl, int rho_slot, int grid) {
        hipLaunchKernelGGL((update_xr_kernel<T, VEC>), dim3(grid), dim3(kBlock), 0, stream, sl.nown / VEC, sl.plane, sl.sc.p, rho_slot, sl.pq.p,
// ... 565 lines not shown
        enum { V_MU = 0, V_R = 1, V_P = 2, V_Z = 3, V_T1 = 4, V_T2 = 5, V_G = 6 };
        const std::vector<int> nopart(slabs.size(), 0);
        auto gather = [&](int sel) {
            for (Slab<T>& sl : slabs)
                hipLaunchKernelGGL((gather_rows_kernel<T>), dim3(1 + (8 * m + kBlock - 1) / kBlock), dim3(kBlock), 0, stream, m, sl.row_ptr.p, sl.ent_node.p,
                                   sl.ent_coef.p, arr(sl, sel), sl.partials.p, 0, sl.red.p);
            allreduce(0, 1 + m);
        };
        auto scatter = [&](int vec, int sel, int accumulate, double scale = 1.0, bool save = false) {
            for (Slab<T>& sl : slabs)
                hipLaunchKernelGGL((scatter_rows_to_nodes_kernel<T>), dim3((sl.n_touched + kBlock - 1) / kBlock + 1), dim3(kBlock), 0, stream, sl.n_touched,
                                   sl.node_id.p, sl.node_ptr.p, sl.ent_row.p, sl.nent_coef.p, mv(sl, vec), accumulate, arr(sl, sel), scale, save ? sl.touched_save.p : (T*)nullptr);
        };
        auto precondition = [&](int init) {
            for (Slab<T>& sl : slabs) {
                apply_Ginv(mv(sl, V_R), mv(sl, V_T1), true, stream);
                hipLaunchKernelGGL(csr_matvec_kernel, dim3((m + kBlock - 1) / kBlock), dim3(kBlock), 0, stream, m, Bptr.p, Bcol.p, Bval.p, mv(sl, V_T1), mv(sl, V_T2));
                apply_Ginv(mv(sl, V_T2), mv(sl, V_Z), true, stream);
                hipLaunchKernelGGL(dual_direction_kernel, dim3(1), dim3(kDualBlock), 0, stream, m, init, mv(sl, V_R), mv(sl, V_Z), mv(sl, V_P), sl.sc.p);
            }
        };
        launch_precond(false, ARR_R, ARR_Z);
        gather(ARR_Z);
        for (Slab<T>& sl : slabs) {
            HIPCHK(hipMemcpyAsync(mv(sl, V_G), sl.red.p + 1, (size_t)m * sizeof(double), hipMemcpyDeviceToDevice, stream));
            if (sl.div_sum_blocks > 0) {
                hipLaunchKernelGGL(finalize_sum_kernel, dim3(1), dim3(kBlock), 0, stream, sl.div_partials.p, sl.div_sum_blocks, sl.pq.p);
                continue;
            }
            const int g = grid_for(sl.nown, 1024);
            hipLaunchKernelGGL((sum_kernel<T>), dim3(g), dim3(kBlock), 0, stream, sl.nown, sl.plane, sl.r.p, sl.partials.p);
            hipLaunchKernelGGL(finalize_sum_kernel, dim3(1), dim3(kBlock), 0, stream, sl.partials.p, g, sl.pq.p);
        }
        allreduce(1, 1);
        for (Slab<T>& sl : slabs) {
            hipLaunchKernelGGL(dual_init_mu_kernel, dim3(1), dim3(kDualBlock), 0, stream, m, sl.pq.p, mv(sl, V_MU), sl.sc.p);
        }
        const bool sparse_ok = total_slabs == 1 && slabs[0].n_act_x > 0;
        const bool dense_S = have_S;
        if (!dense_S)
            for (Slab<T>& sl : slabs) HIPCHK(hipMemsetAsync(sl.p.p, 0, sl.ntot * sizeof(T), stream));
        auto apply_S = [&](int vec) {
            for (Slab<T>& sl : slabs) launch_ginv_matvec<double>(stream, m, m, mp, Sdense.p, mv(sl, vec), sl.red.p + 1);
        };
        if (dense_S) apply_S(V_MU);
        else {
            scatter(V_MU, ARR_P, 0);
            if (sparse_ok) launch_precond_sparse(ARR_P, ARR_Z);
            else launch_precond(false, ARR_P, ARR_Z);
            gather(ARR_Z);
        }
        for (Slab<T>& sl : slabs)
            hipLaunchKernelGGL(dual_init_residual_kernel, dim3(1), dim3(kDualBlock), 0, stream, m, mv(sl, V_G), sl.red.p + 1, mv(sl, V_R), sl.sc.p, 1);
        const bool direct = plan.dual_form == SHM_DUAL_DIRECT && dense_S;
        if (!direct) precondition(1);
        HIPCHK(hipGetLastError());

        SampleTimer tm(st != nullptr, 32, 3);
        int it = 0;
        Residual res;
        bool converged = false, breakdown = false;
        auto finish = [&]() {
            if (gemm_dct()) {
                for (Slab<T>& sl : slabs)
                    hipLaunchKernelGGL((negate_kernel<T>), dim3(grid_for(sl.ntot, 4096)), dim3(kBlock), 0, stream, sl.ntot, sl.r.p, sl.q.p);
                scatter(V_MU, ARR_Q, 1);
                launch_precond(false, ARR_Q, ARR_X);
            } else {
                scatter(V_MU, ARR_R, 1, -1.0, true);
                launch_precond(false, ARR_R, ARR_X, -1.0);
                for (Slab<T>& sl : slabs)
                    hipLaunchKernelGGL((restore_nodes_kernel<T>), dim3((sl.n_touched + kBlock - 1) / kBlock + 1), dim3(kBlock), 0, stream, sl.n_touched, sl.node_id.p,
                                       sl.touched_save.p, sl.r.p);
            }
            gather(ARR_X);
            for (Slab<T>& sl : slabs) hipLaunchKernelGGL(finalize_sum_kernel, dim3(1), dim3(kBlock), 0, stream, sl.red.p + 1, m, sl.sc.p + SC_AXSUM);
            e_pcg.record(stream);
            launch_shift_and_phi();
            e_end.record(stream);
            return fetch_residual();
        };
        bool finished = false;
        if (direct) {
            auto apply_Sinv = [&](const double* w, double* u) { launch_ginv_matvec<double>(stream, m, m, mp, Sinv.p, w, u); };
            const int max_passes = std::min(o.max_iters, 6);
            double rr_prev = -1.;
            while (it < max_passes && !converged && !breakdown) {
                tm.begin();
                tm.mark(0, stream);
                for (Slab<T>& sl : slabs) {
                    apply_Sinv(mv(sl, V_R), mv(sl, V_T1));
                    hipLaunchKernelGGL(dual_bordered_kernel, dim3(1), dim3(kDualBlock), 0, stream, m, mv(sl, V_T1), Sinv_ones.p, (const double*)nullptr, 1, mv(sl, V_MU));
                }
                tm.mark(1, stream);
                apply_S(V_MU);
                for (Slab<T>& sl : slabs)
                    hipLaunchKernelGGL(dual_init_residual_kernel, dim3(1), dim3(kDualBlock), 0, stream, m, mv(sl, V_G), sl.red.p + 1, mv(sl, V_R), sl.sc.p, 0);
                tm.mark(2, stream);
                tm.end();
                it++;
                HIPCHK(hipGetLastError());
                res = finish();
                finished = true;
                if (!res.finite) breakdown = true;
                else if (res.below(o.tol)) converged = true;
                else if (rr_prev >= 0. && res.rr > 0.0625 * rr_prev && res.rr <= 1e-18 * res.rr0) converged = true;
                rr_prev = res.rr;
                log("[shm] dual (direct) pass=%d rel_res=%.3e", it, res.rel());
            }
        }
        while (!direct && it < o.max_iters && !converged && !breakdown) {
            const int batch_end = std::min(o.max_iters, it + check_every);
            for (; it < batch_end; it++) {
                tm.begin();
                if (!dense_S) scatter(V_P, ARR_P, 0);
                tm.mark(0, stream);
                if (dense_S) apply_S(V_P);
                else if (sparse_ok) launch_precond_sparse(ARR_P, ARR_Z);
                else launch_precond(false, ARR_P, ARR_Z);
                tm.mark(1, stream);
                if (!dense_S) gather(ARR_Z);
                for (Slab<T>& sl : slabs)
                    hipLaunchKernelGGL(dual_update_kernel, dim3(1), dim3(kDualBlock), 0, stream, m, sl.red.p + 1, mv(sl, V_P), mv(sl, V_MU), mv(sl, V_R), sl.sc.p);
                precondition(0);
                tm.mark(2, stream);
                tm.end();
            }
            HIPCHK(hipGetLastError());
            res = fetch_residual(SC_RZ);
            if (!res.finite) breakdown = true;
            else if (res.below(o.tol)) converged = true;
            log("[shm] dual it=%d rel_res=%.3e", it, res.rel());
        }
        if (!finished) finish();
        have_phi = true;
        have_div = false;
        if (st) {
            fill_phase_stats(st, clk, e_pcg, e_end, it, res.rel());
            st->shift += h_pinned[SC_AXSUM] / (double)m;
            st->ms_precond_avg = tm.avg(0, 1);
            st->ms_project_avg = tm.avg(1, 2);
            st->kernel_samples = tm.n;
            st->preconditioner = SHM_PRECOND_DCT;
            st->solver = total_slabs > 1 ? SHM_SOLVER_DUAL_SLABS : SHM_SOLVER_DUAL;
            if (direct) {
                st->bytes_per_iter = 2.0 * (double)m * m * sizeof(double);
                st->cg_form = 2;
            } else if (dense_S) {
                st->bytes_per_iter = (double)m * m * (sizeof(double) + 2.0 * sizeof(float));
                st->cg_form = 3;
            } else if (sparse_ok) {
                const double L = dct_lines_for(log2n, (int)sizeof(TP)), tile_bytes = L * n * sizeof(TP);
                const double planes_active = (double)slabs[0].n_act_y / (n / L);
                st->bytes_per_iter = 4.0 * slabs[0].n_act_x * tile_bytes + 4.0 * slabs[0].n_act_y * tile_bytes + 2.0 * planes_active * n * n * sizeof(TP);
            } else {
                st->bytes_per_iter = (double)N * (3.0 * sizeof(T) + 8.0 * sizeof(TP)) - (double)N * sizeof(T);
            }
        }
        throw_loop_end("dual CG", breakdown, converged, it, res, o);
    }

    void solve_gathered(const shm_opts& o, const PlanIn& in, shm_stats* st, SolveClock& clk) {
        Solver<T>& F = *full;
        Slab<T>& fs = F.slabs[0];
        Event e_gather;
        SolveClock fclk;
        fclk.wall0 = clk.wall0;
// ... 381 lines not shown
        if (kb) *kb = slabs.front().k0;
        if (ke) *ke = slabs.back().k1;
    }

    void get_field(shm_field f, double* out) override {
        need_problem();
        HIPCHK(hipSetDevice(cfg.device));
        if ((f == SHM_FIELD_Y0 || f == SHM_FIELD_Y1 || f == SHM_FIELD_Y2) && !have_conv) throw Error(SHM_ERR_STATE, "Y not computed");
        if (f == SHM_FIELD_DIV && !have_div) throw Error(SHM_ERR_STATE, "divergence not computed");
        if (f == SHM_FIELD_PHI && !have_phi) throw Error(SHM_ERR_STATE, "phi not computed");
        copy_owned_to_host((int)f, out);
    }

    void get_field_planes(shm_field f, int ka, int kb, double* out) override {
        need_problem();
        HIPCHK(hipSetDevice(cfg.device));
        if ((f == SHM_FIELD_Y0 || f == SHM_FIELD_Y1 || f == SHM_FIELD_Y2) && !have_conv) throw Error(SHM_ERR_STATE, "Y not computed");
        if (f == SHM_FIELD_DIV && !have_div) throw Error(SHM_ERR_STATE, "divergence not computed");
        if (f == SHM_FIELD_PHI && !have_phi) throw Error(SHM_ERR_STATE, "phi not computed");
        if (ka < slabs.front().k0 || kb > slabs.back().k1 || kb < ka) throw Error(SHM_ERR_INVALID, "plane range outside the planes this process owns");
        copy_planes_to_host((int)f, ka, kb, out);
    }

    void upload_owned(const double* in, int which) {
        std::vector<T> tmp;
        for (Slab<T>& sl : slabs) {
            tmp.assign(sl.ntot, (T)0);
            const int klo = std::max(0, sl.k0 - 1), khi = std::min(n, sl.k1 + 1);
            for (int k = klo; k < khi; k++)
                for (size_t a = 0; a < sl.plane; a++) tmp[(size_t)(k - sl.k0 + 1) * sl.plane + a] = (T)in[(size_t)k * sl.plane + a];
            T* dst = which == 0 ? sl.p.p : which == 1 ? sl.r.p : sl.q.p;
            HIPCHK(hipMemcpyAsync(dst, tmp.data(), sl.ntot * sizeof(T), hipMemcpyHostToDevice, stream));
            HIPCHK(hipStreamSynchronize(stream));
        }
    }

    void apply_laplacian(const double* u, double* out) override {
        need_problem();
        if (cfg.world != 1) throw Error(SHM_ERR_INVALID, "apply_laplacian is a single-process test entry point");
        HIPCHK(hipSetDevice(cfg.device));
        upload_owned(u, 0);
        for (Slab<T>& sl : slabs)
            hipLaunchKernelGGL((laplacian_kernel<T>), dim3(grid_for(sl.nown, 4096)), dim3(kBlock), 0, stream, sl.gp, sl.p.p, sl.q.p);
        HIPCHK(hipGetLastError());
        copy_owned_to_host(SHM_FIELD_PHI, out);
        have_phi = false;
        iso_idx_valid = false;
        ray_bricks_valid = false;
        redist_valid = false;
    }

    void set_phi(const double* phi) override {
        need_problem();
        if (cfg.world != 1) throw Error(SHM_ERR_INVALID, "set_phi is a single-process test entry point");
        HIPCHK(hipSetDevice(cfg.device));
        upload_owned(phi, 2);
        have_phi = true;
        iso_idx_valid = false;
        cmp_valid = false;
        ray_bricks_valid = false;
        redist_valid = false;
    }

    void get_constraints(int64_t* nodes, double* coeffs, int32_t* m_out) override {
        need_problem();
        build_rows();
        for (int r = 0; r < m; r++)
            for (int e = 0; e < 8; e++) {
                nodes[8 * (size_t)r + e] = rows[r].nodes[e];
                coeffs[8 * (size_t)r + e] = rows[r].coeffs[e];
            }
        *m_out = m;
    }

    void get_schur(double* out, int32_t* m_out) override {
        need_problem();
        if (cfg.world != 1) throw Error(SHM_ERR_INVALID, "get_schur is a single-process test entry point");
        HIPCHK(hipSetDevice(cfg.device));
        build_constraints(plan_inputs(nullptr), Plan());
        *m_out = m;
        if (!have_S) throw Error(SHM_ERR_STATE, "no explicit Schur complement for this problem (several slabs, more than 16384 rows, or n = 2^k where the plan applies S through the grid: n > 512, or the estimate of plan_explicit_S without SHM_DUAL_DENSE_S_ALWAYS)");
        HIPCHK(hipMemcpy2DAsync(out, (size_t)m * sizeof(double), Sdense.p, (size_t)mp * sizeof(double), (size_t)m * sizeof(double), (size_t)m, hipMemcpyDeviceToHost, stream2));
        HIPCHK(hipStreamSynchronize(stream2));
    }

    void apply_projector(double* v) override {
        need_problem();
        if (cfg.world != 1) throw Error(SHM_ERR_INVALID, "apply_projector is a single-process test entry point");
        HIPCHK(hipSetDevice(cfg.device));
        build_constraints(plan_inputs(nullptr), Plan());
        upload_owned(v, 1);
        std::vector<int> nparts(slabs.size(), 0);
        launch_projection(nparts);
        HIPCHK(hipGetLastError());
        have_div = true;
        copy_owned_to_host(SHM_FIELD_DIV, v);
        have_div = false;
    }

    std::vector<double> iso_vertices;
    std::vector<int64_t> iso_triangles;

    void isosurface(double iso, int method, int64_t* nv, int64_t* nt) override {
        need_problem();
        if (method != SHM_ISO_MARCHING_CUBES && method != SHM_ISO_MARCHING_TETS) throw Error(SHM_ERR_INVALID, fmt("isosurface: unknown method %d", method));
        const bool mc = method == SHM_ISO_MARCHING_CUBES;
        if (!have_phi) throw Error(SHM_ERR_STATE, "no phi: shm_grid_solve has not completed");
        HIPCHK(hipSetDevice(cfg.device));
        halo_exchange(ARR_Q);
        iso_vertices.clear();
        iso_triangles.clear();
        std::unordered_map<uint64_t, int64_t> weld;
        for (Slab<T>& sl : slabs) {
            IsoParams P;
            P.n = n; P.nzl = sl.nzl; P.k0 = sl.k0;
            for (int a = 0; a < 3; a++) P.bbox_min[a] = bbox_min[a];
            P.cell = cell; P.iso = iso;
            DevArray<unsigned long long> counter, keys, sortk;
            DevArray<double> pos;
            counter.alloc(1);
            HIPCHK(hipMemsetAsync(counter.p, 0, sizeof(unsigned long long), stream));
            const size_t ncells = (size_t)(n - 1) * (n - 1) * (size_t)std::max(0, std::min(sl.nzl, n - 1 - sl.k0));
            const int grid = grid_for(ncells, 8192);
            if (mc) hipLaunchKernelGGL((iso_mc_kernel<T, false>), dim3(grid), dim3(kBlock), 0, stream, P, sl.q.p, counter.p, (double*)nullptr, (unsigned long long*)nullptr,
                                       (unsigned long long*)nullptr, 0ULL);
            else hipLaunchKernelGGL((iso_kernel<T, false>), dim3(grid), dim3(kBlock), 0, stream, P, sl.q.p, counter.p, (double*)nullptr, (unsigned long long*)nullptr,
                                    (unsigned long long*)nullptr, 0ULL);
            unsigned long long ntri = 0;
            HIPCHK(hipMemcpyAsync(&ntri, counter.p, sizeof ntri, hipMemcpyDeviceToHost, stream));
            HIPCHK(hipStreamSynchronize(stream));
            if (ntri == 0) continue;
            pos.alloc(ntri * 9);
            keys.alloc(ntri * 3);
            sortk.alloc(ntri);
            HIPCHK(hipMemsetAsync(counter.p, 0, sizeof(unsigned long long), stream));
            if (mc) hipLaunchKernelGGL((iso_mc_kernel<T, true>), dim3(grid), dim3(kBlock), 0, stream, P, sl.q.p, counter.p, pos.p, keys.p, sortk.p, ntri);
            else hipLaunchKernelGGL((iso_kernel<T, true>), dim3(grid), dim3(kBlock), 0, stream, P, sl.q.p, counter.p, pos.p, keys.p, sortk.p, ntri);
            HIPCHK(hipGetLastError());
            std::vector<double> hpos(ntri * 9);
            std::vector<unsigned long long> hkeys(ntri * 3), hsort(ntri);
            HIPCHK(hipMemcpyAsync(hpos.data(), pos.p, hpos.size() * sizeof(double), hipMemcpyDeviceToHost, stream));
            HIPCHK(hipMemcpyAsync(hkeys.data(), keys.p, hkeys.size() * sizeof(unsigned long long), hipMemcpyDeviceToHost, stream));
            HIPCHK(hipMemcpyAsync(hsort.data(), sortk.p, hsort.size() * sizeof(unsigned long long), hipMemcpyDeviceToHost, stream));
            HIPCHK(hipStreamSynchronize(stream));
            std::vector<size_t> order(ntri);
            for (size_t a = 0; a < ntri; a++) order[a] = a;
            std::sort(order.begin(), order.end(), [&](size_t x, size_t y) { return hsort[x] < hsort[y]; });
            for (size_t a : order)
                for (int c = 0; c < 3; c++) {
                    auto ins = weld.insert({hkeys[a * 3 + c], (int64_t)(iso_vertices.size() / 3)});
                    if (ins.second)
                        for (int b = 0; b < 3; b++) iso_vertices.push_back(hpos[a * 9 + c * 3 + b]);
                    iso_triangles.push_back(ins.first->second);
                }
        }
        if (nv) *nv = (int64_t)(iso_vertices.size() / 3);
        if (nt) *nt = (int64_t)(iso_triangles.size() / 3);
    }

    static constexpr int64_t kSampleChunk = (int64_t)1 << 20;
    DevArray<unsigned long long> d_sample_count;
    DevArray<double> smp_dev[2];
    void* smp_pinned[2] = {nullptr, nullptr};
    int64_t smp_cap = 0;
    std::unique_ptr<Event> smp_done[2];

// ... 990 lines not shown
```

signed-heat-3d_amd/grid_abi.py:

```python
from __future__ import annotations

import ctypes as C
import os

import numpy as np

SHM_F64, SHM_F32 = 64, 32
_HERE = os.path.dirname(os.path.abspath(__file__))

STATUS_NAMES = {0: "SHM_OK", 1: "SHM_ERR_INVALID", 2: "SHM_ERR_HIP", 3: "SHM_ERR_NOMEM", 4: "SHM_ERR_BREAKDOWN",
                5: "SHM_ERR_NOCONV", 6: "SHM_ERR_RCCL", 7: "SHM_ERR_STATE", 8: "SHM_ERR_SINGULAR"}

ABI_SYMBOLS = ["shm_grid_owned_planes", "shm_grid_create", "shm_grid_destroy", "shm_grid_last_error", "shm_grid_abi_version", "shm_grid_set_problem",
               "shm_grid_solve", "shm_grid_get_phi", "shm_grid_compute_distance", "shm_grid_run_conv", "shm_grid_run_conv_arith", "shm_grid_run_divergence",
               "shm_grid_get_field", "shm_grid_get_field_planes", "shm_grid_apply_laplacian", "shm_grid_set_phi", "shm_grid_get_constraints", "shm_grid_get_schur", "shm_grid_apply_projector", "shm_grid_apply_preconditioner", "shm_grid_isosurface", "shm_grid_isosurface_ex", "shm_grid_get_isosurface",
               "shm_grid_isosurface_indexed", "shm_grid_get_isosurface_indexed", "shm_grid_get_isosurface_indexed_device",
               "shm_grid_label_mesh_device", "shm_grid_isosurface_components", "shm_grid_get_isosurface_components", "shm_grid_isosurface_keep_components",
               "shm_grid_sample", "shm_grid_sample_device", "shm_grid_raycast", "shm_grid_raycast_device",
               "shm_grid_redistance", "shm_grid_get_redistanced", "shm_grid_get_redistanced_device", "shm_grid_redistance_exact", "shm_grid_isosurface_indexed_psi",
               "shm_grid_closest_point", "shm_grid_closest_point_device",
               "shm_grid_audit_step1", "shm_comm_unique_id", "shm_plan_slab", "shm_step1_plane_weights", "shm_plan_slab_weighted"]


class ShmError(RuntimeError):
    def __init__(self, status, message):
        super().__init__("%s: %s" % (STATUS_NAMES.get(status, status), message))
        self.status = status


class _Config(C.Structure):
    _fields_ = [("device", C.c_int32), ("precision", C.c_int32), ("local_slabs", C.c_int32), ("rank", C.c_int32),
                ("world", C.c_int32), ("verbose", C.c_int32), ("rccl_unique_id", C.c_void_p), ("slab_plan", C.c_int32)]


class _Sources(C.Structure):
    _fields_ = [("S", C.c_int64), ("pos", C.c_void_p), ("wnormal", C.c_void_p), ("area", C.c_void_p), ("lam", C.c_double)]


class _Grid(C.Structure):
    _fields_ = [("n", C.c_int32), ("bbox_min", C.c_double * 3), ("cell", C.c_double)]


class _Opts(C.Structure):
    _fields_ = [("fast_integration", C.c_int32), ("scrub_nonfinite", C.c_int32), ("tol", C.c_double), ("max_iters", C.c_int32),
                ("check_every", C.c_int32), ("preconditioner", C.c_int32), ("solver", C.c_int32), ("step1_arith", C.c_int32),
                ("dual_form", C.c_int32), ("step1_budget", C.c_double)]


class ShmStats(C.Structure):
    _fields_ = [("n", C.c_int32), ("m", C.c_int32), ("S", C.c_int64), ("iters", C.c_int32), ("rel_residual", C.c_double),
                ("shift", C.c_double), ("ms_conv", C.c_double), ("ms_div", C.c_double), ("ms_setup", C.c_double), ("ms_wait_setup", C.c_double),
                ("ms_pcg", C.c_double), ("ms_shift", C.c_double), ("ms_total", C.c_double), ("ms_stencil_avg", C.c_double),
                ("ms_update_xr_avg", C.c_double), ("ms_project_avg", C.c_double), ("ms_update_p_avg", C.c_double),
                ("ms_precond_avg", C.c_double), ("kernel_samples", C.c_int32), ("preconditioner", C.c_int32),
                ("solver", C.c_int32), ("bytes_per_iter", C.c_double), ("cg_form", C.c_int32), ("pairs_fp64", C.c_double), ("pairs_fp32", C.c_double), ("conv_launches", C.c_int32), ("pairs_redone", C.c_double)]

    def as_dict(self):
        return {k: getattr(self, k) for k, _ in self._fields_}


class ShmStep1Audit(C.Structure):
    _fields_ = [("n_audited", C.c_int64), ("n_not_owned", C.c_int64), ("n_nonfinite", C.c_int64), ("n_out_of_zone", C.c_int64),
                ("n_finite_mismatch", C.c_int64), ("max_dy", C.c_double), ("worst_node", C.c_int64), ("worst_ratio", C.c_double), ("min_ratio", C.c_double),
                ("budget", C.c_double), ("step1_arith", C.c_int32), ("within_budget", C.c_int32), ("ms", C.c_double)]

    def as_dict(self):
        return {k: getattr(self, k) for k, _ in self._fields_}


class ShmRedistanceStats(C.Structure):
    _fields_ = [("n_frozen", C.c_int64), ("n_reached", C.c_int64), ("n_nonfinite", C.c_int64), ("n_block_updates", C.c_int64), ("n_rounds", C.c_int32),
                ("reserved", C.c_int32), ("max_abs", C.c_double), ("isovalue", C.c_double), ("band", C.c_double), ("ms", C.c_double)]

    def as_dict(self):
        return {k: getattr(self, k) for k, _ in self._fields_ if k != "reserved"}


class ShmRedistanceExactStats(C.Structure):
    _fields_ = [("n_vertices", C.c_int64), ("n_triangles", C.c_int64), ("n_reached", C.c_int64), ("n_candidate_pairs", C.c_int64), ("max_abs", C.c_double),
                ("isovalue", C.c_double), ("band", C.c_double), ("ms", C.c_double)]

    def as_dict(self):
        return {k: getattr(self, k) for k, _ in self._fields_}


class ShmIsoComponent(C.Structure):
    _fields_ = [("first_vertex", C.c_int64), ("n_vertices", C.c_int64), ("n_triangles", C.c_int64), ("area", C.c_double), ("volume", C.c_double),
                ("lo", C.c_double * 3), ("hi", C.c_double * 3), ("touches_box", C.c_int32), ("reserved", C.c_int32)]


ISO_COMPONENT_DTYPE = np.dtype([("first_vertex", "<i8"), ("n_vertices", "<i8"), ("n_triangles", "<i8"), ("area", "<f8"), ("volume", "<f8"),
                                ("lo", "<f8", (3,)), ("hi", "<f8", (3,)), ("touches_box", "<i4"), ("reserved", "<i4")])
assert ISO_COMPONENT_DTYPE.itemsize == C.sizeof(ShmIsoComponent) == 96


def largest_components_mask(comps, keep_largest=None, min_triangles=None):
    nc = len(comps)
    mask = np.ones(nc, dtype=np.uint8)
    if min_triangles is not None:
        mask &= (comps["n_triangles"] >= int(min_triangles)).astype(np.uint8)
    if keep_largest is not None:
        order = np.lexsort((comps["first_vertex"], -comps["n_triangles"]))
        top = np.zeros(nc, dtype=np.uint8)
        top[order[:max(0, int(keep_largest))]] = 1
        mask &= top
    return mask


def lib_path():
    return os.environ.get("SHM_GRID_LIB") or os.path.join(_HERE, "lib", "libshm_grid.so")


_LIB = None


def load_library():
    global _LIB
    if _LIB is not None:
        return _LIB
    path = lib_path()
    if not os.path.exists(path):
        raise OSError("libshm_grid.so not built: run `python -c 'import __graft_entry__ as g; g.build()'` (%s)" % path)
    lib = C.CDLL(path)
    lib.shm_grid_last_error.restype = C.c_char_p
    lib.shm_grid_last_error.argtypes = [C.c_void_p]
    lib.shm_grid_create.argtypes = [C.POINTER(_Config), C.POINTER(C.c_void_p)]
    lib.shm_grid_destroy.argtypes = [C.c_void_p]
    lib.shm_grid_destroy.restype = None
    lib.shm_grid_set_problem.argtypes = [C.c_void_p, C.POINTER(_Sources), C.POINTER(_Grid)]
    lib.shm_grid_solve.argtypes = [C.c_void_p, C.POINTER(_Opts), C.POINTER(ShmStats)]
    lib.shm_grid_get_phi.argtypes = [C.c_void_p, C.c_void_p, C.POINTER(C.c_int32), C.POINTER(C.c_int32)]
    lib.shm_grid_compute_distance.argtypes = [C.c_void_p, C.POINTER(_Sources), C.POINTER(_Grid), C.POINTER(_Opts), C.c_void_p,
                                              C.POINTER(ShmStats)]
    lib.shm_grid_run_conv.argtypes = [C.c_void_p]
    lib.shm_grid_run_conv_arith.argtypes = [C.c_void_p, C.c_int32]
    lib.shm_grid_run_divergence.argtypes = [C.c_void_p, C.c_int32]
    lib.shm_grid_get_field.argtypes = [C.c_void_p, C.c_int, C.c_void_p]
    lib.shm_grid_get_field_planes.argtypes = [C.c_void_p, C.c_int, C.c_int32, C.c_int32, C.c_void_p]
    lib.shm_grid_apply_laplacian.argtypes = [C.c_void_p, C.c_void_p, C.c_void_p]
    lib.shm_grid_set_phi.argtypes = [C.c_void_p, C.c_void_p]
    lib.shm_grid_get_constraints.argtypes = [C.c_void_p, C.c_void_p, C.c_void_p, C.POINTER(C.c_int32)]
    lib.shm_grid_get_schur.argtypes = [C.c_void_p, C.c_void_p, C.POINTER(C.c_int32)]
    lib.shm_grid_apply_projector.argtypes = [C.c_void_p, C.c_void_p]
    lib.shm_grid_apply_preconditioner.argtypes = [C.c_void_p, C.c_void_p, C.c_void_p]
    lib.shm_grid_isosurface.argtypes = [C.c_void_p, C.c_double, C.POINTER(C.c_int64), C.POINTER(C.c_int64)]
    lib.shm_grid_isosurface_ex.argtypes = [C.c_void_p, C.c_double, C.c_int32, C.POINTER(C.c_int64), C.POINTER(C.c_int64)]
    lib.shm_grid_get_isosurface.argtypes = [C.c_void_p, C.c_void_p, C.c_void_p]
    lib.shm_grid_sample.argtypes = [C.c_void_p, C.c_int64, C.c_void_p, C.c_void_p, C.c_void_p, C.POINTER(C.c_int64)]
    lib.shm_grid_sample_device.argtypes = [C.c_void_p, C.c_int64, C.c_void_p, C.c_void_p, C.c_void_p, C.POINTER(C.c_int64)]
    if hasattr(lib, "shm_grid_isosurface_indexed"):
        lib.shm_grid_isosurface_indexed.argtypes = [C.c_void_p, C.c_double, C.POINTER(C.c_int64), C.POINTER(C.c_int64)]
        lib.shm_grid_get_isosurface_indexed.argtypes = [C.c_void_p, C.c_void_p, C.c_void_p]
        lib.shm_grid_get_isosurface_indexed_device.argtypes = [C.c_void_p, C.c_void_p, C.c_void_p]
    if hasattr(lib, "shm_grid_label_mesh_device"):
        lib.shm_grid_label_mesh_device.argtypes = [C.c_void_p, C.c_int64, C.c_int64, C.c_void_p, C.c_void_p, C.POINTER(C.c_int64)]
        lib.shm_grid_isosurface_components.argtypes = [C.c_void_p, C.POINTER(C.c_int64)]
        lib.shm_grid_get_isosurface_components.argtypes = [C.c_void_p, C.c_void_p, C.c_void_p, C.c_void_p]
        lib.shm_grid_isosurface_keep_components.argtypes = [C.c_void_p, C.c_void_p, C.POINTER(C.c_int64), C.POINTER(C.c_int64)]
    if hasattr(lib, "shm_grid_audit_step1"):
        lib.shm_grid_audit_step1.argtypes = [C.c_void_p, C.c_int64, C.c_void_p, C.c_void_p, C.c_void_p, C.POINTER(ShmStep1Audit)]
        lib.shm_audit_sample_nodes.argtypes = [C.c_int32, C.c_int32, C.c_int32, C.c_int64, C.c_uint64, C.c_void_p]
        lib.shm_audit_sample_nodes.restype = C.c_int64
    if hasattr(lib, "shm_grid_raycast"):
        lib.shm_grid_raycast.argtypes = [C.c_void_p, C.c_int64, C.c_void_p, C.c_void_p, C.c_double, C.c_double, C.c_double, C.c_void_p, C.c_void_p, C.POINTER(C.c_int64)]
        lib.shm_grid_raycast_device.argtypes = lib.shm_grid_raycast.argtypes
    if hasattr(lib, "shm_grid_redistance"):
        lib.shm_grid_redistance.argtypes = [C.c_void_p, C.c_double, C.c_double, C.POINTER(ShmRedistanceStats)]
        lib.shm_grid_get_redistanced.argtypes = [C.c_void_p, C.c_void_p]
        lib.shm_grid_get_redistanced_device.argtypes = [C.c_void_p, C.c_void_p]
    if hasattr(lib, "shm_grid_redistance_exact"):
        lib.shm_grid_redistance_exact.argtypes = [C.c_void_p, C.c_double, C.c_double, C.POINTER(ShmRedistanceExactStats)]
        lib.shm_grid_isosurface_indexed_psi.argtypes = [C.c_void_p, C.c_double, C.POINTER(C.c_int64), C.POINTER(C.c_int64)]
    if hasattr(lib, "shm_grid_closest_point"):
        lib.shm_grid_closest_point.argtypes = [C.c_void_p, C.c_int64, C.c_void_p, C.c_double, C.c_void_p, C.c_void_p, C.c_void_p, C.POINTER(C.c_int64)]
        lib.shm_grid_closest_point_device.argtypes = lib.shm_grid_closest_point.argtypes
    lib.shm_grid_owned_planes.argtypes = [C.c_void_p, C.POINTER(C.c_int32), C.POINTER(C.c_int32)]
    lib.shm_comm_unique_id.argtypes = [C.c_void_p]
    lib.shm_plan_slab.argtypes = [C.c_int32, C.c_int32, C.c_int32, C.POINTER(C.c_int32), C.POINTER(C.c_int32)]
    lib.shm_plan_slab.restype = None
    lib.shm_step1_plane_weights.argtypes = [C.c_void_p, C.c_void_p, C.c_int32, C.c_void_p]
    lib.shm_plan_slab_weighted.argtypes = [C.c_int32, C.c_int32, C.c_int32, C.c_void_p, C.c_int32, C.POINTER(C.c_int32), C.POINTER(C.c_int32)]
    lib.shm_plan_slab_weighted.restype = None
    _LIB = lib
    return lib


def plan_slab(n, nslabs, slab):
    lib = load_library()
    k0, k1 = C.c_int32(), C.c_int32()
    lib.shm_plan_slab(n, nslabs, slab, C.byref(k0), C.byref(k1))
    return k0.value, k1.value


def audit_sample_nodes(n, k_begin, k_end, count, seed=0):
    lib = load_library()
    out = np.empty(max(0, min(int(count), max(0, int(k_end) - int(k_begin)) * int(n) * int(n))), dtype=np.int64)
    got = lib.shm_audit_sample_nodes(int(n), int(k_begin), int(k_end), int(out.size), int(seed) & 0xFFFFFFFFFFFFFFFF, out.ctypes.data) if out.size else 0
    return out[:got]


def step1_plane_weights(pos, wnormal, lam, n, bbox_min, cell, precision=SHM_F64):
    lib = load_library()
    pos, wn = _f64(pos).reshape(-1), _f64(wnormal).reshape(-1)
    area = np.zeros(pos.size // 3)
    src = _Sources(pos.size // 3, pos.ctypes.data, wn.ctypes.data, area.ctypes.data, float(lam))
    g = _Grid(int(n), (C.c_double * 3)(*[float(x) for x in bbox_min]), float(cell))
    w = np.zeros(int(n))
    rc = lib.shm_step1_plane_weights(C.byref(src), C.byref(g), int(precision), w.ctypes.data)
    if rc != 0:
        raise ShmError(rc, "shm_step1_plane_weights: invalid argument")
    return w


def plan_slab_weighted(n, nslabs, slab, weights, granule):
    lib = load_library()
    w = _f64(weights)
    k0, k1 = C.c_int32(), C.c_int32()
    lib.shm_plan_slab_weighted(int(n), int(nslabs), int(slab), w.ctypes.data, int(granule), C.byref(k0), C.byref(k1))
    return k0.value, k1.value


def comm_unique_id():
    lib = load_library()
    buf = C.create_string_buffer(128)
    rc = lib.shm_comm_unique_id(buf)
# ... 50 lines not shown
        self._chk(self._lib.shm_grid_set_problem(self._h, C.byref(src), C.byref(g)))
        self.n, self.S, self.cell = int(n), S, float(cell)

    def owned_planes(self):
        k0, k1 = C.c_int32(), C.c_int32()
        self._chk(self._lib.shm_grid_owned_planes(self._h, C.byref(k0), C.byref(k1)))
        return k0.value, k1.value

    PRECOND = {"auto": 0, "none": 1, "dct": 2}

    SOLVER = {"auto": 0, "primal": 1, "dual": 2, "dual_slabs": 3}

    STEP1 = {"auto": 0, "exact_f64": 1, "reference_f64": 2}

    DUAL_FORM = {"auto": 0, "direct": 1, "explicit_s_cg": 2, "through_grid": 3}

    def solve(self, tol=0.0, max_iters=0, check_every=0, scrub=True, fast=False, allow_noconv=False, precond="auto", solver="auto", step1="auto",
              dual_form="auto", step1_budget=0.0):
        o = _Opts(int(fast), int(scrub), float(tol), int(max_iters), int(check_every), self.PRECOND[precond], self.SOLVER[solver], self.STEP1[step1],
                  self.DUAL_FORM[dual_form], float(step1_budget))
        st = ShmStats()
        self._chk(self._lib.shm_grid_solve(self._h, C.byref(o), C.byref(st)), allow=(5,) if allow_noconv else ())
        return st

    def _owned_count(self):
        k0, k1 = self.owned_planes()
        return (k1 - k0) * self.n * self.n

    def get_phi(self):
        out = np.empty(self._owned_count(), dtype=np.float64)
        k0, k1 = C.c_int32(), C.c_int32()
        self._chk(self._lib.shm_grid_get_phi(self._h, out.ctypes.data, C.byref(k0), C.byref(k1)))
        return out, (k0.value, k1.value)

    def run_conv(self, step1="auto"):
        if step1 == "auto":
            self._chk(self._lib.shm_grid_run_conv(self._h))
        else:
            self._chk(self._lib.shm_grid_run_conv_arith(self._h, self.STEP1[step1]))

    def run_divergence(self, scrub=True):
        self._chk(self._lib.shm_grid_run_divergence(self._h, int(scrub)))

    def get_field(self, which):
        out = np.empty(self._owned_count(), dtype=np.float64)
        self._chk(self._lib.shm_grid_get_field(self._h, int(which), out.ctypes.data))
        return out

    def get_field_planes(self, which, k_begin, k_end):
        out = np.empty((int(k_end) - int(k_begin)) * self.n * self.n, dtype=np.float64)
        self._chk(self._lib.shm_grid_get_field_planes(self._h, int(which), int(k_begin), int(k_end), out.ctypes.data))
        return out

    def apply_laplacian(self, u):
        u = _f64(u).reshape(-1)
        out = np.empty_like(u)
        self._chk(self._lib.shm_grid_apply_laplacian(self._h, u.ctypes.data, out.ctypes.data))
        return out

    def set_phi(self, phi):
        if phi is None:
            self._chk(self._lib.shm_grid_set_phi(self._h, None))
            return
        phi = _f64(phi).reshape(-1)
        if self.n and phi.size != self.n ** 3:
            raise ValueError("set_phi: phi must hold n^3 = %d values, got %d" % (self.n ** 3, phi.size))
        self._chk(self._lib.shm_grid_set_phi(self._h, phi.ctypes.data))

    def get_constraints(self):
        nodes = np.empty(8 * self.S, dtype=np.int64)
        coeffs = np.empty(8 * self.S, dtype=np.float64)
        m = C.c_int32()
        self._chk(self._lib.shm_grid_get_constraints(self._h, nodes.ctypes.data, coeffs.ctypes.data, C.byref(m)))
        return nodes[:8 * m.value].reshape(-1, 8).copy(), coeffs[:8 * m.value].reshape(-1, 8).copy()

    def get_schur(self):
        m = len(self.get_constraints()[0])
        out = np.empty((m, m), dtype=np.float64)
        mm = C.c_int32(0)
        self._chk(self._lib.shm_grid_get_schur(self._h, out.ctypes.data, C.byref(mm)))
        assert mm.value == m
        return out

    def apply_projector(self, v):
        v = _f64(v).reshape(-1).copy()
        self._chk(self._lib.shm_grid_apply_projector(self._h, v.ctypes.data))
        return v

    def apply_preconditioner(self, v):
        v = _f64(v).reshape(-1)
        out = np.empty_like(v)
        self._chk(self._lib.shm_grid_apply_preconditioner(self._h, v.ctypes.data, out.ctypes.data))
        return out

    ISO_METHOD = {"marching_cubes": 0, "marching_tets": 1}

    def isosurface(self, isovalue=0.0, method="marching_cubes"):
        nv, nt = C.c_int64(), C.c_int64()
        if method == "marching_cubes":
            self._chk(self._lib.shm_grid_isosurface(self._h, float(isovalue), C.byref(nv), C.byref(nt)))
        else:
            self._chk(self._lib.shm_grid_isosurface_ex(self._h, float(isovalue), self.ISO_METHOD[method], C.byref(nv), C.byref(nt)))
        V = np.empty((nv.value, 3), dtype=np.float64)
        F = np.empty((nt.value, 3), dtype=np.int64)
        self._chk(self._lib.shm_grid_get_isosurface(self._h, V.ctypes.data, F.ctypes.data))
        return V, F

    def isosurface_indexed(self, isovalue=0.0, device=False, keep_largest=None, min_triangles=None):
        nv, nt = C.c_int64(), C.c_int64()
        self._chk(self._lib.shm_grid_isosurface_indexed(self._h, float(isovalue), C.byref(nv), C.byref(nt)))
        if keep_largest is not None or min_triangles is not None:
            nv.value, nt.value = self.isosurface_keep(largest_components_mask(self.isosurface_components(), keep_largest, min_triangles))
        return self.get_isosurface_indexed(nv.value, nt.value, device)

    def get_isosurface_indexed(self, nv, nt, device=False):
        if not device:
            V = np.empty((nv, 3), dtype=np.float64)
            F = np.empty((nt, 3), dtype=np.int64)
            self._chk(self._lib.shm_grid_get_isosurface_indexed(self._h, V.ctypes.data if nv else None, F.ctypes.data if nt else None))
            return V, F
        import torch
        if not torch.cuda.is_available():
            raise RuntimeError("isosurface_indexed: torch sees no HIP device (was torch imported after libshm_grid.so was loaded? import it first)")
        dev = torch.device("cuda", self.device)
        V = torch.empty((nv, 3), dtype=torch.float64 if self.precision == SHM_F64 else torch.float32, device=dev)
        F = torch.empty((nt, 3), dtype=torch.int64, device=dev)
        self._chk(self._lib.shm_grid_get_isosurface_indexed_device(self._h, V.data_ptr() if nv else None, F.data_ptr() if nt else None))
        return V, F

    def label_mesh_device(self, triangles, nv):
        import torch
        if not torch.cuda.is_available():
            raise RuntimeError("label_mesh_device: torch sees no HIP device (was torch imported after libshm_grid.so was loaded? import it first)")
        if triangles.dtype != torch.int64 or not triangles.is_contiguous() or triangles.numel() % 3:
            raise ValueError("label_mesh_device: triangles must be a contiguous int64 tensor of 3 nt indices")
        nt = triangles.numel() // 3
        root = torch.empty(int(nv), dtype=torch.int64, device=triangles.device)
        if triangles.is_cuda:
            torch.cuda.current_stream(triangles.device).synchronize()
        nc = C.c_int64()
        self._chk(self._lib.shm_grid_label_mesh_device(self._h, int(nv), nt, triangles.data_ptr() if nt else None, root.data_ptr() if nv else None, C.byref(nc)))
        return root, nc.value

    def isosurface_components(self, labels=False):
        nc = C.c_int64()
        self._chk(self._lib.shm_grid_isosurface_components(self._h, C.byref(nc)))
        comps = np.zeros(nc.value, dtype=ISO_COMPONENT_DTYPE)
        if not labels:
            self._chk(self._lib.shm_grid_get_isosurface_components(self._h, comps.ctypes.data if nc.value else None, None, None))
            return comps
        self._chk(self._lib.shm_grid_get_isosurface_components(self._h, comps.ctypes.data if nc.value else None, None, None))
        nv, nt = int(comps["n_vertices"].sum()), int(comps["n_triangles"].sum())
        tc = np.empty(nt, dtype=np.int64)
        vc = np.empty(nv, dtype=np.int64)
        self._chk(self._lib.shm_grid_get_isosurface_components(self._h, comps.ctypes.data if nc.value else None, tc.ctypes.data if nt else None,
                                                               vc.ctypes.data if nv else None))
        return comps, tc, vc

    def isosurface_keep(self, mask):
        mask = np.ascontiguousarray(np.asarray(mask) != 0, dtype=np.uint8).reshape(-1)
        nv, nt = C.c_int64(), C.c_int64()
        self._chk(self._lib.shm_grid_isosurface_keep_components(self._h, mask.ctypes.data if mask.size else None, C.byref(nv), C.byref(nt)))
        return nv.value, nt.value

    def sample(self, points, grad=False):
        pts = _f64(points).reshape(-1, 3)
# ... 172 lines not shown
```

Baseline: 701.0 million.

## Factor the dense Schur complement with blocked LDL instead of full Gauss-Jordan inversion

Adds a blocked LDL^T factorisation of the explicit Schur complement S. It reuses the Gauss-Jordan step kernel through a templated include, and adds triangular and diagonal solve kernels driven by an LdlPlan. When plan.s_factor is set, S is factored rather than fully inverted, and applications of S^-1 become forward and backward triangular solves. This is meant to cut the cubic work of a full inversion roughly in half, at the cost of a sequence of small launches per solve instead of one matvec. A spd_solve test entry point is also exposed.

```diff
diff --git a/include/shm_grid.h b/include/shm_grid.h
--- a/include/shm_grid.h
+++ b/include/shm_grid.h
@@ -130,6 +130,7 @@
 shm_status shm_grid_set_phi(shm_solver* s, const double* phi );
 shm_status shm_grid_get_constraints(shm_solver* s, int64_t* nodes, double* coeffs, int32_t* m);
 shm_status shm_grid_get_schur(shm_solver* s, double* out, int32_t* m);
+shm_status shm_grid_spd_solve(shm_solver* s, const double* S, int32_t m, const double* rhs, int32_t form, double* u, int32_t* flag);
 shm_status shm_grid_apply_projector(shm_solver* s, double* v);
 
 shm_status shm_grid_apply_preconditioner(shm_solver* s, const double* v, double* out);
diff --git a/signed-heat-3d_amd/csrc/shm_gj_step.inc.h b/signed-heat-3d_amd/csrc/shm_gj_step.inc.h
--- /dev/null
+++ b/signed-heat-3d_amd/csrc/shm_gj_step.inc.h
@@ -0,0 +1,187 @@
+static __global__ __launch_bounds__(kBlock) __attribute__((amdgpu_waves_per_eu(SHM_GJ_STEP_WAVES, SHM_GJ_STEP_WAVES))) void SHM_GJ_STEP_NAME(
+    double* __restrict__ G, int ld, int nb, int k, const double* __restrict__ Rp , const double* __restrict__ Cp ,
+    double* __restrict__ Rn, double* __restrict__ Cn, int* __restrict__ flag, int prio SHM_GJ_STEP_EXTRA_PARAM) {
+    constexpr int MODE = SHM_GJ_STEP_MODE;
+
+    __shared__ double smem[kGjStepLds];
+    static_assert(kGjStepLds >= kGjUpdateLds && kGjStepScratch >= 8 * kGJ, "LDS carve");
+    if (prio) __builtin_amdgcn_s_setprio(3);
+    const int nN = MODE == kGjStepLdl ? shm::ldl_panel_count(nb, k) : (k < nb ? nb : 0);
+    if ((int)blockIdx.x >= nN) {
+#if SHM_GJ_STEP_MODE == 1
+        const int nS = shm::ldl_store_count(nb, k);
+        if ((int)blockIdx.x < nN + nS) {
+            double(*xt)[kGJ + 1] = reinterpret_cast<double(*)[kGJ + 1]>(smem);
+            const size_t ob = (size_t)(k + (int)blockIdx.x - nN) * kGJ, oc = (size_t)(k - 1) * kGJ;
+            for (int t = threadIdx.x; t < kGJ * kGJ; t += kBlock) {
+                const int i = t / kGJ, j = t % kGJ;
+                xt[i][j] = Rp[(size_t)i * ld + ob + j];
+            }
+            __syncthreads();
+            for (int t = threadIdx.x; t < kGJ * kGJ; t += kBlock) {
+                const int i = t / kGJ, j = t % kGJ;
+                G[(ob + i) * ld + oc + j] = xt[j][i];
+            }
+            return;
+        }
+        {
+            int ti, tj;
+            shm::ldl_update_tile(k, blockIdx.x - (unsigned)(nN + nS), ti, tj);
+            gj_update_tile(G, ld, ti, tj, -1, Rp, 0, Cp, kGJ, 0, kGJ, smem);
+            return;
+        }
+#endif
+        int bi, bj;
+        gj_tri_decode(blockIdx.x - (unsigned)nN, bi, bj);
+        if (k < nb) {
+            if (bi >= k) bi += 1;
+            if (bj >= k) bj += 1;
+        }
+        gj_update_tile(G, ld, bi, bj, k - 1, Rp, 0, Cp, kGJ, 0, kGJ, smem);
+        return;
+    }
+    double(*x)[kGJ + 1] = reinterpret_cast<double(*)[kGJ + 1]>(smem);
+    double* scratch = smem + kGJ * (kGJ + 1);
+    double(*prow)[kGJ + 1] = reinterpret_cast<double(*)[kGJ + 1]>(scratch);
+#if SHM_GJ_STEP_MODE == 1
+    const int b = k + (int)blockIdx.x;
+#else
+    const int b = blockIdx.x;
+#endif
+    const bool below = b >= k;
+    const int bi = below ? b : k, bj = below ? k : b;
+    const size_t o = (size_t)k * kGJ, ob = (size_t)b * kGJ, oi = (size_t)bi * kGJ, oj = (size_t)bj * kGJ;
+    const int lane = threadIdx.x & 63, w = threadIdx.x >> 6, wr = w >> 1, wc = w & 1, l15 = lane & 15, l4 = lane >> 4;
+    const int ty = threadIdx.x >> 4, tx = threadIdx.x & 15;
+    double r[4][4];
+    double* Cb = Cn + ob * kGJ;
+    if (k > 0) {
+        auto product = [&](gj_f64x4(&acc)[2][2], size_t orow, size_t ocol) {
+#pragma unroll
+            for (int a = 0; a < 2; a++)
+#pragma unroll
+                for (int c = 0; c < 2; c++) acc[a][c] = gj_f64x4{0., 0., 0., 0.};
+#pragma unroll 1
+            for (int g = 0; g < 2; g++) {
+                double af[8][2], bf[8][2];
+#pragma unroll
+                for (int u = 0; u < 8; u++) {
+                    const int kk = 32 * g + 4 * u + l4;
+#pragma unroll
+                    for (int a = 0; a < 2; a++) af[u][a] = Cp[(orow + wr * 32 + a * 16 + l15) * kGJ + kk];
+#pragma unroll
+                    for (int c = 0; c < 2; c++) bf[u][c] = Rp[(size_t)kk * ld + ocol + wc * 32 + c * 16 + l15];
+                }
+#pragma unroll
+                for (int u = 0; u < 8; u++)
+#pragma unroll
+                    for (int a = 0; a < 2; a++)
+#pragma unroll
+                        for (int c = 0; c < 2; c++) acc[a][c] = __builtin_amdgcn_mfma_f64_16x16x4f64(af[u][a], bf[u][c], acc[a][c], 0, 0, 0);
+            }
+        };
+        {
+            gj_f64x4 accp[2][2];
+            product(accp, o, o);
+#pragma unroll
+            for (int a = 0; a < 2; a++)
+#pragma unroll
+                for (int c = 0; c < 2; c++)
+#pragma unroll
+                    for (int q = 0; q < 4; q++) {
+                        const size_t row = wr * 32 + a * 16 + l4 + 4 * q, col = wc * 32 + c * 16 + l15;
+                        x[row][col] = G[(o + row) * ld + o + col] - accp[a][c][q];
+                    }
+        }
+        gj_f64x4 accx[2][2];
+        product(accx, oi, oj);
+        __syncthreads();
+#pragma unroll
+        for (int a = 0; a < 4; a++)
+#pragma unroll
+            for (int c = 0; c < 4; c++) r[a][c] = x[ty * 4 + a][tx * 4 + c];
+        __syncthreads();
+        const double keep = b == k - 1 ? 0. : 1.;
+#pragma unroll
+        for (int a = 0; a < 2; a++)
+#pragma unroll
+            for (int c = 0; c < 2; c++)
+#pragma unroll
+                for (int q = 0; q < 4; q++) {
+                    const size_t row = wr * 32 + a * 16 + l4 + 4 * q, col = wc * 32 + c * 16 + l15;
+                    x[row][col] = G[(oi + row) * ld + oj + col] * keep - accx[a][c][q];
+                }
+    } else {
+        for (int t = threadIdx.x; t < kGJ * kGJ; t += kBlock) {
+            const int i = t / kGJ, j = t % kGJ;
+            x[i][j] = G[(oi + i) * ld + oj + j];
+        }
+#pragma unroll
+        for (int a = 0; a < 4; a++)
+#pragma unroll
+            for (int c = 0; c < 4; c++) r[a][c] = G[(o + ty * 4 + a) * ld + o + tx * 4 + c];
+    }
+    __syncthreads();
+    for (int t = threadIdx.x; t < kGJ * kGJ; t += kBlock) {
+        const int i = t / kGJ, j = t % kGJ;
+        Cb[i * kGJ + j] = below ? x[i][j] : -x[j][i];
+    }
+    gj_invert64_scalar<4, SHM_GJ_STEP_PAIRS != 0>(r, scratch, flag);
+#if SHM_GJ_STEP_MODE == 1
+    if (b == k) {
+#pragma unroll
+        for (int a = 0; a < 4; a++)
+#pragma unroll
+            for (int c = 0; c < 4; c++) Pd[(size_t)k * kGJ * kGJ + (ty * 4 + a) * kGJ + tx * 4 + c] = r[a][c];
+        return;
+    }
+#endif
+    if (b == k) {
+#pragma unroll
+        for (int a = 0; a < 4; a++)
+#pragma unroll
+            for (int c = 0; c < 4; c++) Rn[(size_t)(ty * 4 + a) * ld + ob + tx * 4 + c] = r[a][c];
+        return;
+    }
+    double pa[2][kGJ / 4];
+#pragma unroll
+    for (int pass = 0; pass < 8; pass++) {
+        __syncthreads();
+        if ((ty >> 1) == pass) {
+#pragma unroll
+            for (int a = 0; a < 4; a++)
+#pragma unroll
+                for (int c = 0; c < 4; c++) prow[(ty & 1) * 4 + a][tx * 4 + c] = r[a][c];
+        }
+        __syncthreads();
+        if (wr == (pass >> 2) && (l15 >> 3) == (pass & 1)) {
+#pragma unroll
+            for (int s4 = 0; s4 < kGJ / 4; s4++) pa[(pass >> 1) & 1][s4] = prow[l15 & 7][4 * s4 + l4];
+        }
+    }
+    gj_f64x4 acc[2][2];
+#pragma unroll
+    for (int a = 0; a < 2; a++)
+#pragma unroll
+        for (int c = 0; c < 2; c++) acc[a][c] = gj_f64x4{0., 0., 0., 0.};
+#pragma unroll
+    for (int s4 = 0; s4 < kGJ / 4; s4++) {
+        const int kk = 4 * s4 + l4;
+        double bf[2];
+#pragma unroll
+        for (int c = 0; c < 2; c++) {
+            const int j = wc * 32 + c * 16 + l15;
+            bf[c] = (b > k) ? x[j][kk] : x[kk][j];
+        }
+#pragma unroll
+        for (int a = 0; a < 2; a++)
+#pragma unroll
+            for (int c = 0; c < 2; c++) acc[a][c] = __builtin_amdgcn_mfma_f64_16x16x4f64(pa[a][s4], bf[c], acc[a][c], 0, 0, 0);
+    }
+#pragma unroll
+    for (int a = 0; a < 2; a++)
+#pragma unroll
+        for (int c = 0; c < 2; c++)
+#pragma unroll
+            for (int q = 0; q < 4; q++) Rn[(size_t)(wr * 32 + a * 16 + l4 + 4 * q) * ld + ob + wc * 32 + c * 16 + l15] = acc[a][c][q];
+}
diff --git a/signed-heat-3d_amd/csrc/shm_grid.hip b/signed-heat-3d_amd/csrc/shm_grid.hip
--- a/signed-heat-3d_amd/csrc/shm_grid.hip
+++ b/signed-heat-3d_amd/csrc/shm_grid.hip
@@ -188,6 +188,12 @@
         s->impl->get_schur(out, m);
     });
 }
+shm_status shm_grid_spd_solve(shm_solver* s, const double* S, int32_t m, const double* rhs, int32_t form, double* u, int32_t* flag) {
+    return guard(s, [&] {
+        if (!S || !rhs || !u || !flag) throw shm::Error(SHM_ERR_INVALID, "null argument");
+        s->impl->spd_solve(S, m, rhs, form, u, flag);
+    });
+}
 shm_status shm_grid_apply_projector(shm_solver* s, double* v) {
     return guard(s, [&] {
         if (!v) throw shm::Error(SHM_ERR_INVALID, "null argument");
diff --git a/signed-heat-3d_amd/csrc/shm_host.hip.h b/signed-heat-3d_amd/csrc/shm_host.hip.h
--- a/signed-heat-3d_amd/csrc/shm_host.hip.h
+++ b/signed-heat-3d_amd/csrc/shm_host.hip.h
@@ -515,6 +515,7 @@
     virtual void apply_projector(double*) = 0;
     virtual void apply_preconditioner(const double*, double*) = 0;
     virtual void get_schur(double*, int32_t*) = 0;
+    virtual void spd_solve(const double*, int32_t, const double*, int32_t, double*, int32_t*) = 0;
     virtual void isosurface(double, int, int64_t*, int64_t*) = 0;
     virtual void get_isosurface(double*, int64_t*) = 0;
     virtual void sample(int64_t, const double*, double*, double*, int64_t*) = 0;
diff --git a/signed-heat-3d_amd/csrc/shm_kernels.hip.h b/signed-heat-3d_amd/csrc/shm_kernels.hip.h
--- a/signed-heat-3d_amd/csrc/shm_kernels.hip.h
+++ b/signed-heat-3d_amd/csrc/shm_kernels.hip.h
@@ -5,6 +5,7 @@
 #include <type_traits>
 
 #include "shm_constraints.h"
+#include "shm_ldl_plan.h"
 #include "shm_mc_table.h"
 
 namespace shm {
@@ -1565,154 +1566,91 @@
 #endif
 constexpr int kGjStepScratch = 8 * (kGJ + 1);
 constexpr int kGjStepLds = kGJ * (kGJ + 1) + kGjStepScratch;
-static __global__ __launch_bounds__(kBlock) __attribute__((amdgpu_waves_per_eu(SHM_GJ_STEP_WAVES, SHM_GJ_STEP_WAVES))) void gj_step_kernel(
-    double* __restrict__ G, int ld, int nb, int k, const double* __restrict__ Rp , const double* __restrict__ Cp ,
-    double* __restrict__ Rn, double* __restrict__ Cn, int* __restrict__ flag, int prio) {
-    __shared__ double smem[kGjStepLds];
-    static_assert(kGjStepLds >= kGjUpdateLds && kGjStepScratch >= 8 * kGJ, "LDS carve");
+enum GjStepMode : int { kGjStepInverse = 0, kGjStepLdl = 1 };
+#define SHM_GJ_STEP_NAME gj_step_kernel
+#define SHM_GJ_STEP_MODE 0
+#define SHM_GJ_STEP_EXTRA_PARAM
+#include "shm_gj_step.inc.h"
+#undef SHM_GJ_STEP_NAME
+#undef SHM_GJ_STEP_MODE
+#undef SHM_GJ_STEP_EXTRA_PARAM
+#define SHM_GJ_STEP_NAME gj_ldl_step_kernel
+#define SHM_GJ_STEP_MODE 1
+#define SHM_GJ_STEP_EXTRA_PARAM , double* __restrict__ Pd
+#include "shm_gj_step.inc.h"
+#undef SHM_GJ_STEP_NAME
+#undef SHM_GJ_STEP_MODE
+#undef SHM_GJ_STEP_EXTRA_PARAM
+
+static __global__ __launch_bounds__(kBlock) void ldl_tri_kernel(double* __restrict__ F, int ld, shm::LdlPlan plan, int t, double* __restrict__ panels, int pld, int prio) {
+    __shared__ double smem[kGjUpdateLds];
     if (prio) __builtin_amdgcn_s_setprio(3);
-    const int nN = k < nb ? nb : 0;
-    if ((int)blockIdx.x >= nN) {
-        int bi, bj;
-        gj_tri_decode(blockIdx.x - (unsigned)nN, bi, bj);
-        if (k < nb) {
-            if (bi >= k) bi += 1;
-            if (bj >= k) bj += 1;
-        }
-        gj_update_tile(G, ld, bi, bj, k - 1, Rp, 0, Cp, kGJ, 0, kGJ, smem);
+    const int q = blockIdx.y, s = plan.len(q), xw = blockIdx.x;
+    double* Fq = F + ((size_t)plan.start[q] * kGJ) * ld + (size_t)plan.start[q] * kGJ;
+    double* pan = panels + (size_t)q * 2 * kGJ * pld;
+    if (xw < shm::ldl_tri_compute_count(t)) {
+        if (t >= s) return;
+        const int j = xw;
+        const double* Crow = pan + (size_t)(t & 1) * kGJ * pld - (size_t)t * kGJ * pld;
+        gj_update_tile(Fq, ld, t, j, -1, Fq, (j + 1) * kGJ, Crow, pld, (j + 1) * kGJ, (t - j - 1) * kGJ, smem);
         return;
     }
-    double(*x)[kGJ + 1] = reinterpret_cast<double(*)[kGJ + 1]>(smem);
-    double* scratch = smem + kGJ * (kGJ + 1);
-    double(*prow)[kGJ + 1] = reinterpret_cast<double(*)[kGJ + 1]>(scratch);
-    const int b = blockIdx.x;
-    const bool below = b >= k;
-    const int bi = below ? b : k, bj = below ? k : b;
-    const size_t o = (size_t)k * kGJ, ob = (size_t)b * kGJ, oi = (size_t)bi * kGJ, oj = (size_t)bj * kGJ;
-    const int lane = threadIdx.x & 63, w = threadIdx.x >> 6, wr = w >> 1, wc = w & 1, l15 = lane & 15, l4 = lane >> 4;
-    const int ty = threadIdx.x >> 4, tx = threadIdx.x & 15;
-    double r[4][4];
-    double* Cb = Cn + ob * kGJ;
-    if (k > 0) {
-        auto product = [&](gj_f64x4(&acc)[2][2], size_t orow, size_t ocol) {
-#pragma unroll
-            for (int a = 0; a < 2; a++)
-#pragma unroll
-                for (int c = 0; c < 2; c++) acc[a][c] = gj_f64x4{0., 0., 0., 0.};
-#pragma unroll 1
-            for (int g = 0; g < 2; g++) {
-                double af[8][2], bf[8][2];
-#pragma unroll
-                for (int u = 0; u < 8; u++) {
-                    const int kk = 32 * g + 4 * u + l4;
-#pragma unroll
-                    for (int a = 0; a < 2; a++) af[u][a] = Cp[(orow + wr * 32 + a * 16 + l15) * kGJ + kk];
-#pragma unroll
-                    for (int c = 0; c < 2; c++) bf[u][c] = Rp[(size_t)kk * ld + ocol + wc * 32 + c * 16 + l15];
-                }
-#pragma unroll
-                for (int u = 0; u < 8; u++)
-#pragma unroll
-                    for (int a = 0; a < 2; a++)
-#pragma unroll
-                        for (int c = 0; c < 2; c++) acc[a][c] = __builtin_amdgcn_mfma_f64_16x16x4f64(af[u][a], bf[u][c], acc[a][c], 0, 0, 0);
-            }
-        };
-        {
-            gj_f64x4 accp[2][2];
-            product(accp, o, o);
-#pragma unroll
-            for (int a = 0; a < 2; a++)
-#pragma unroll
-                for (int c = 0; c < 2; c++)
-#pragma unroll
-                    for (int q = 0; q < 4; q++) {
-                        const size_t row = wr * 32 + a * 16 + l4 + 4 * q, col = wc * 32 + c * 16 + l15;
-                        x[row][col] = G[(o + row) * ld + o + col] - accp[a][c][q];
-                    }
-        }
-        gj_f64x4 accx[2][2];
-        product(accx, oi, oj);
-        __syncthreads();
-#pragma unroll
-        for (int a = 0; a < 4; a++)
-#pragma unroll
-            for (int c = 0; c < 4; c++) r[a][c] = x[ty * 4 + a][tx * 4 + c];
-        __syncthreads();
-        const double keep = b == k - 1 ? 0. : 1.;
-#pragma unroll
-        for (int a = 0; a < 2; a++)
-#pragma unroll
-            for (int c = 0; c < 2; c++)
-#pragma unroll
-                for (int q = 0; q < 4; q++) {
-                    const size_t row = wr * 32 + a * 16 + l4 + 4 * q, col = wc * 32 + c * 16 + l15;
-                    x[row][col] = G[(oi + row) * ld + oj + col] * keep - accx[a][c][q];
-                }
-    } else {
-        for (int t = threadIdx.x; t < kGJ * kGJ; t += kBlock) {
-            const int i = t / kGJ, j = t % kGJ;
-            x[i][j] = G[(oi + i) * ld + oj + j];
-        }
-#pragma unroll
-        for (int a = 0; a < 4; a++)
-#pragma unroll
-            for (int c = 0; c < 4; c++) r[a][c] = G[(o + ty * 4 + a) * ld + o + tx * 4 + c];
-    }
-    __syncthreads();
-    for (int t = threadIdx.x; t < kGJ * kGJ; t += kBlock) {
-        const int i = t / kGJ, j = t % kGJ;
-        Cb[i * kGJ + j] = below ? x[i][j] : -x[j][i];
-    }
-    gj_invert64_scalar<4, SHM_GJ_STEP_PAIRS != 0>(r, scratch, flag);
-    if (b == k) {
-#pragma unroll
-        for (int a = 0; a < 4; a++)
-#pragma unroll
-            for (int c = 0; c < 4; c++) Rn[(size_t)(ty * 4 + a) * ld + ob + tx * 4 + c] = r[a][c];
-        return;
-    }
-    double pa[2][kGJ / 4];
-#pragma unroll
-    for (int pass = 0; pass < 8; pass++) {
-        __syncthreads();
-        if ((ty >> 1) == pass) {
-#pragma unroll
-            for (int a = 0; a < 4; a++)
-#pragma unroll
-                for (int c = 0; c < 4; c++) prow[(ty & 1) * 4 + a][tx * 4 + c] = r[a][c];
-        }
-        __syncthreads();
-        if (wr == (pass >> 2) && (l15 >> 3) == (pass & 1)) {
-#pragma unroll
-            for (int s4 = 0; s4 < kGJ / 4; s4++) pa[(pass >> 1) & 1][s4] = prow[l15 & 7][4 * s4 + l4];
-        }
-    }
-    gj_f64x4 acc[2][2];
-#pragma unroll
-    for (int a = 0; a < 2; a++)
-#pragma unroll
-        for (int c = 0; c < 2; c++) acc[a][c] = gj_f64x4{0., 0., 0., 0.};
-#pragma unroll
-    for (int s4 = 0; s4 < kGJ / 4; s4++) {
-        const int kk = 4 * s4 + l4;
-        double bf[2];
-#pragma unroll
-        for (int c = 0; c < 2; c++) {
-            const int j = wc * 32 + c * 16 + l15;
-            bf[c] = (b > k) ? x[j][kk] : x[kk][j];
-        }
-#pragma unroll
-        for (int a = 0; a < 2; a++)
-#pragma unroll
-            for (int c = 0; c < 2; c++) acc[a][c] = __builtin_amdgcn_mfma_f64_16x16x4f64(pa[a][s4], bf[c], acc[a][c], 0, 0, 0);
-    }
-#pragma unroll
-    for (int a = 0; a < 2; a++)
-#pragma unroll
-        for (int c = 0; c < 2; c++)
-#pragma unroll
-            for (int q = 0; q < 4; q++) Rn[(size_t)(wr * 32 + a * 16 + l4 + 4 * q) * ld + ob + wc * 32 + c * 16 + l15] = acc[a][c][q];
+    if (t + 1 >= s) return;
+    const int c = xw - shm::ldl_tri_compute_count(t) + 1;
+    double* dst = pan + (size_t)((t + 1) & 1) * kGJ * pld + (size_t)c * kGJ;
+    const double* src = Fq + ((size_t)(t + 1) * kGJ) * ld + (size_t)c * kGJ;
+    for (int e = threadIdx.x; e < kGJ * kGJ; e += kBlock) {
+        const int i = e / kGJ, jj = e % kGJ;
+        dst[(size_t)i * pld + jj] = src[(size_t)i * ld + jj];
+    }
+}
+
+template <int U>
+__global__ __launch_bounds__(kBlock) void ldl_matvec_kernel(int op, int row0, int c0, int c1, int ld, const double* __restrict__ F, const double* __restrict__ a,
+                                                           const double* __restrict__ x, double* __restrict__ u) {
+    __shared__ double lds[8];
+    const int row = row0 + blockIdx.x;
+    if (op == shm::kLdlLower) c1 = min(c1, row / kGJ * kGJ);
+    if (op == shm::kLdlUpper) c0 = max(c0, (row / kGJ + 1) * kGJ);
+    const double* g = F + (size_t)row * ld;
+    double s = 0.;
+    for (int cc = c0; cc < c1; cc += U * kBlock * 4) {
+        double gv[U][4];
+#pragma unroll
+        for (int e = 0; e < U; e++) {
+            const int c = cc + (threadIdx.x + e * kBlock) * 4;
+            if (c < c1) {
+                *reinterpret_cast<double2*>(gv[e]) = *reinterpret_cast<const double2*>(g + c);
+                *reinterpret_cast<double2*>(gv[e] + 2) = *reinterpret_cast<const double2*>(g + c + 2);
+            }
+        }
+#pragma unroll
+        for (int e = 0; e < U; e++) {
+            const int c = cc + (threadIdx.x + e * kBlock) * 4;
+            if (c < c1) {
+                double d = gv[e][0] * x[c];
+                if (c + 1 < c1) d += gv[e][1] * x[c + 1];
+                if (c + 2 < c1) d += gv[e][2] * x[c + 2];
+                if (c + 3 < c1) d += gv[e][3] * x[c + 3];
+                s += d;
+            }
+        }
+    }
+    s = block_sum(s, lds);
+    if (threadIdx.x == 0) u[row] = a[row] - s;
+}
+static __global__ __launch_bounds__(kBlock) void ldl_diag_kernel(int m, const double* __restrict__ Pd, const double* __restrict__ y, double* __restrict__ z) {
+    const int blk = blockIdx.x, i = threadIdx.x >> 2, part = threadIdx.x & 3, row = blk * kGJ + i;
+    const double* p = Pd + (size_t)blk * kGJ * kGJ + (size_t)i * kGJ + part * 16;
+    double s = 0.;
+#pragma unroll
+    for (int c = 0; c < 16; c++) {
+        const int col = blk * kGJ + part * 16 + c;
+        if (col < m) s += p[c] * y[col];
+    }
+    s += __shfl_xor(s, 1, 64);
+    s += __shfl_xor(s, 2, 64);
+    if (part == 0 && row < m) z[row] = s;
 }
 
 static __global__ __launch_bounds__(kBlock) void gj_mirror_kernel(double* __restrict__ G_, int ld, GjBatch Bt = GjBatch{nullptr, nullptr, nullptr, nullptr, nullptr, nullptr, nullptr}) {
diff --git a/signed-heat-3d_amd/csrc/shm_ldl_plan.h b/signed-heat-3d_amd/csrc/shm_ldl_plan.h
--- /dev/null
+++ b/signed-heat-3d_amd/csrc/shm_ldl_plan.h
@@ -0,0 +1,136 @@
+#pragma once
+#include <cmath>
+#include <cstdint>
+
+#ifdef __HIPCC__
+#define SHM_LDL_HD __host__ __device__ __forceinline__
+#else
+#define SHM_LDL_HD inline
+#endif
+
+namespace shm {
+
+constexpr int kLdlTile = 64;
+constexpr int kLdlMaxSuper = 4;
+
+SHM_LDL_HD bool ldl_applies(int nb) { return nb >= 1 && nb < 64; }
+
+struct LdlPlan {
+    int nb;
+    int B;
+    int start[kLdlMaxSuper + 1];
+    SHM_LDL_HD int len(int q) const { return start[q + 1] - start[q]; }
+    SHM_LDL_HD int max_len() const { return len(0); }
+};
+
+SHM_LDL_HD LdlPlan ldl_plan(int nb) {
+    LdlPlan p;
+    p.nb = nb;
+    p.B = (nb + 3) / 4 < kLdlMaxSuper ? (nb + 3) / 4 : kLdlMaxSuper;
+    if (p.B < 1) p.B = 1;
+    int at = 0;
+    for (int q = 0; q <= kLdlMaxSuper; q++) {
+        p.start[q] = at;
+        if (q < p.B) at += nb / p.B + (q < nb % p.B ? 1 : 0);
+    }
+    return p;
+}
+
+SHM_LDL_HD void ldl_tri_decode(unsigned t, int& bi, int& bj) {
+    int r = (int)((sqrt(8.0 * (double)t + 1.0) - 1.0) * 0.5);
+    while ((unsigned)r * (unsigned)(r + 1) / 2 > t) r--;
+    while ((unsigned)(r + 1) * (unsigned)(r + 2) / 2 <= t) r++;
+    bi = r;
+    bj = (int)(t - (unsigned)r * (unsigned)(r + 1) / 2);
+}
+
+SHM_LDL_HD int ldl_panel_count(int nb, int k) { return nb - k; }
+SHM_LDL_HD int ldl_store_count(int nb, int k) { return k == 0 ? 0 : nb - k; }
+SHM_LDL_HD int ldl_update_count(int nb, int k) { return k == 0 ? 0 : (nb - k - 1) * (nb - k) / 2; }
+SHM_LDL_HD void ldl_update_tile(int k, unsigned idx, int& bi, int& bj) {
+    ldl_tri_decode(idx, bi, bj);
+    bi += k + 1;
+    bj += k + 1;
+}
+
+SHM_LDL_HD int ldl_tri_launches(const LdlPlan& p) { return p.max_len() >= 3 ? p.max_len() - 1 : 0; }
+SHM_LDL_HD int ldl_tri_compute_count(int t) { return t - 1; }
+SHM_LDL_HD int ldl_tri_copy_count(int t) { return t; }
+SHM_LDL_HD int ldl_tri_grid(int t) { return ldl_tri_compute_count(t) + ldl_tri_copy_count(t); }
+
+enum LdlOp : int { kLdlRect = 0, kLdlLower = 1, kLdlUpper = 2, kLdlDiag = 3 };
+enum LdlVec : int { kLdlW = 0 , kLdlY = 1, kLdlT = 2, kLdlZ = 3, kLdlU = 4  };
+struct LdlStep {
+    int op;
+    int rb0, rb1;
+    int cb0, cb1;
+    int a, x, u;
+};
+SHM_LDL_HD int ldl_solve_steps(const LdlPlan& p) { return 4 * p.B - 1; }
+SHM_LDL_HD LdlStep ldl_solve_step(const LdlPlan& p, int i) {
+    LdlStep s;
+    const int nf = 2 * p.B - 1;
+    if (i < nf) {
+        const int q = (i + 1) / 2;
+        s.rb0 = p.start[q];
+        s.rb1 = p.start[q + 1];
+        if (q > 0 && (i & 1)) {
+            s.op = kLdlRect; s.cb0 = 0; s.cb1 = p.start[q]; s.a = kLdlW; s.x = kLdlY; s.u = kLdlT;
+        } else {
+            s.op = kLdlLower; s.cb0 = s.rb0; s.cb1 = s.rb1; s.a = s.x = q == 0 ? kLdlW : kLdlT; s.u = kLdlY;
+        }
+    } else if (i == nf) {
+        s.op = kLdlDiag; s.rb0 = s.cb0 = 0; s.rb1 = s.cb1 = p.nb; s.a = s.x = kLdlY; s.u = kLdlZ;
+    } else {
+        const int j = i - nf - 1, q = p.B - 1 - (j + 1) / 2;
+        s.rb0 = p.start[q];
+        s.rb1 = p.start[q + 1];
+        if (q < p.B - 1 && (j & 1)) {
+            s.op = kLdlRect; s.cb0 = p.start[q + 1]; s.cb1 = p.nb; s.a = kLdlZ; s.x = kLdlU; s.u = kLdlT;
+        } else {
+            s.op = kLdlUpper; s.cb0 = s.rb0; s.cb1 = s.rb1; s.a = s.x = q == p.B - 1 ? kLdlZ : kLdlT; s.u = kLdlU;
+        }
+    }
+    return s;
+}
+
+SHM_LDL_HD int64_t gj_tile_products(int nb) {
+    const int64_t n = nb;
+    return 2 * n * (n - 1)
+           + n * (n - 1)
+           + (n - 1) * (n - 1) * n / 2
+           + n * (n + 1) / 2;
+}
+SHM_LDL_HD int64_t ldl_elim_tile_products(int nb) {
+    const int64_t n = nb;
+    return n * (n - 1)
+           + n * (n - 1) / 2
+           + (n - 2) * (n - 1) * n / 6;
+}
+SHM_LDL_HD int64_t ldl_tri_tile_products(const LdlPlan& p) {
+    int64_t c = 0;
+    for (int q = 0; q < p.B; q++) {
+        const int64_t s = p.len(q);
+        c += s * (s - 1) * (s - 2) / 6;
+    }
+    return c;
+}
+SHM_LDL_HD int64_t ldl_tile_products(const LdlPlan& p) { return ldl_elim_tile_products(p.nb) + ldl_tri_tile_products(p); }
+constexpr int64_t kLdlTileBytes = (int64_t)kLdlTile * kLdlTile * 8;
+SHM_LDL_HD int64_t gj_tiles_written(int nb) {
+    const int64_t n = nb;
+    return 2 * n * n + (n - 1) * (n - 1) * n / 2 + n * (n + 1) / 2;
+}
+SHM_LDL_HD int64_t ldl_tiles_written(const LdlPlan& p) {
+    const int64_t n = p.nb;
+    int64_t c = n * (n + 1) / 2  + n * (n - 1) / 2  + n * (n + 1) / 2  + (n - 2) * (n - 1) * n / 6;
+    for (int q = 0; q < p.B; q++) {
+        const int64_t s = p.len(q);
+        if (s >= 3) c += (s - 1) * (s - 2) ;
+    }
+    return c;
+}
+SHM_LDL_HD int64_t gj_bytes(int nb) { return kLdlTileBytes * 2 * (gj_tile_products(nb) + gj_tiles_written(nb)); }
+SHM_LDL_HD int64_t ldl_bytes(const LdlPlan& p) { return kLdlTileBytes * 2 * (ldl_tile_products(p) + ldl_tiles_written(p)); }
+
+}
diff --git a/signed-heat-3d_amd/csrc/shm_plan.h b/signed-heat-3d_amd/csrc/shm_plan.h
--- a/signed-heat-3d_amd/csrc/shm_plan.h
+++ b/signed-heat-3d_amd/csrc/shm_plan.h
@@ -3,8 +3,10 @@
 #include <cmath>
 #include <cstdint>
 #include <cstdlib>
+#include <cstring>
 
 #include "../../include/shm_grid.h"
+#include "shm_ldl_plan.h"
 
 namespace shm {
 
@@ -15,6 +17,7 @@
     bool no_direct = false;
     bool no_dense_s = false;
     bool dense_s_always = false;
+    int s_form = 0;
     int tl_min_m = 6144;
 };
 template <typename Get> PlanKnobs plan_knobs(Get knob) {
@@ -22,9 +25,13 @@
     k.no_direct = knob("SHM_DUAL_NO_DIRECT") != nullptr;
     k.no_dense_s = knob("SHM_DUAL_NO_DENSE_S") != nullptr;
     k.dense_s_always = knob("SHM_DUAL_DENSE_S_ALWAYS") != nullptr;
+    const char* s_form = knob("SHM_S_FORM");
+    if (s_form != nullptr) k.s_form = std::strcmp(s_form, "invert") == 0 ? 1 : std::strcmp(s_form, "factor") == 0 ? 2 : 0;
     if (knob("SHM_TL_MIN_M")) k.tl_min_m = atoi(knob("SHM_TL_MIN_M"));
     return k;
 }
+
+constexpr bool kSFactorDefault = true;
 
 struct PlanIn {
     bool f64 = true;
@@ -53,6 +60,7 @@
     int dual_form = SHM_DUAL_THROUGH_GRID;
     bool explicit_S = false;
     bool two_level = false;
+    bool s_factor = false;
     double est_setup_ms = -1., est_step1_ms = -1.;
 };
 
@@ -137,6 +145,7 @@
     p.explicit_S = plan_explicit_S(in, m, direct);
     p.dual_form = direct ? SHM_DUAL_DIRECT : p.explicit_S ? SHM_DUAL_EXPLICIT_S_CG : SHM_DUAL_THROUGH_GRID;
     p.two_level = !direct && m > in.knobs.tl_min_m;
+    p.s_factor = direct && (in.knobs.s_form == 2 || (in.knobs.s_form == 0 && kSFactorDefault)) && ldl_applies((m + kLdlTile - 1) / kLdlTile);
 }
 
 inline const char* plan_path_name(PlanPath path) {
diff --git a/signed-heat-3d_amd/csrc/shm_solver.hip.h b/signed-heat-3d_amd/csrc/shm_solver.hip.h
--- a/signed-heat-3d_amd/csrc/shm_solver.hip.h
+++ b/signed-heat-3d_amd/csrc/shm_solver.hip.h
@@ -150,6 +150,7 @@
     std::vector<int> h_rowX;
     bool have_S = false;
     DevArray<double> Sinv, Sinv_ones ;
+    DevArray<double> ldlP, ldlPanels, ldlWork;
     PlanIn plan_in;
     Plan plan;
     double conv_est_total_ms = 1e30;
@@ -1205,6 +1206,41 @@
         if (nb > 1) hipLaunchKernelGGL(gj_mirror_kernel, dim3((unsigned)((size_t)nb * (nb - 1) / 2)), dim3(kBlock), 0, stream, M, mp);
         HIPCHK(hipGetLastError());
     }
+    void enqueue_ldl_factor(double* M, int mp, DevArray<double>& Pd, DevArray<double>& panels) {
+        hipStream_t stream = stream2;
+        const int nb = mp / kGJ;
+        const LdlPlan lp = ldl_plan(nb);
+        gjR.alloc((size_t)2 * kGJ * mp);
+        gjC.alloc((size_t)2 * mp * kGJ);
+        gjFlag.alloc(2);
+        Pd.alloc((size_t)nb * kGJ * kGJ);
+        HIPCHK(hipMemsetAsync(gjFlag.p, 0, sizeof(int), stream));
+        for (int k = 0; k < nb; k++) {
+            const unsigned grid = (unsigned)(ldl_panel_count(nb, k) + ldl_store_count(nb, k) + ldl_update_count(nb, k));
+            double* Rn = gjR.p + (size_t)(k & 1) * kGJ * mp;
+            double* Cn = gjC.p + (size_t)(k & 1) * mp * kGJ;
+            const double* Rp = gjR.p + (size_t)((k + 1) & 1) * kGJ * mp;
+            const double* Cp = gjC.p + (size_t)((k + 1) & 1) * mp * kGJ;
+            hipLaunchKernelGGL(gj_ldl_step_kernel, dim3(grid), dim3(kBlock), 0, stream, M, mp, nb, k, Rp, Cp, Rn, Cn, gjFlag.p, plan.setup_prio, Pd.p);
+        }
+        const int pld = lp.max_len() * kGJ;
+        panels.alloc((size_t)lp.B * 2 * kGJ * pld);
+        for (int t = 1; t <= ldl_tri_launches(lp); t++)
+            hipLaunchKernelGGL(ldl_tri_kernel, dim3((unsigned)ldl_tri_grid(t), (unsigned)lp.B), dim3(kBlock), 0, stream, M, mp, lp, t, panels.p, pld, plan.setup_prio);
+        if (nb > 1) hipLaunchKernelGGL(gj_mirror_kernel, dim3((unsigned)((size_t)nb * (nb - 1) / 2)), dim3(kBlock), 0, stream, M, mp);
+        HIPCHK(hipGetLastError());
+    }
+    void apply_ldl(hipStream_t st, int m, int mp, const double* F, const double* Pd, double* work, const double* w, double* u) {
+        const LdlPlan lp = ldl_plan(mp / kGJ);
+        auto vec = [&](int v) -> double* { return v == kLdlW ? const_cast<double*>(w) : v == kLdlU ? u : work + (size_t)(v - kLdlY) * mp; };
+        for (int i = 0; i < ldl_solve_steps(lp); i++) {
+            const LdlStep s = ldl_solve_step(lp, i);
+            const int r0 = s.rb0 * kGJ, r1 = std::min(s.rb1 * kGJ, m), c0 = s.cb0 * kGJ, c1 = std::min(s.cb1 * kGJ, m);
+            if (r1 <= r0) continue;
+            if (s.op == kLdlDiag) hipLaunchKernelGGL(ldl_diag_kernel, dim3((unsigned)((m + kGJ - 1) / kGJ)), dim3(kBlock), 0, st, m, Pd, vec(s.x), vec(s.u));
+            else hipLaunchKernelGGL(ldl_matvec_kernel<4>, dim3((unsigned)(r1 - r0)), dim3(kBlock), 0, st, s.op, r0, c0, c1, mp, F, vec(s.a), vec(s.x), vec(s.u));
+        }
+    }
     void enqueue_invert_G() {
         const int mp = ginv_ld;
         enqueue_gj_invert(Ginv.p, mp);
@@ -1327,10 +1363,14 @@
             Sinv.alloc((size_t)mp * mp);
             HIPCHK(hipMemcpyAsync(Sinv.p, Sdense.p, (size_t)mp * mp * sizeof(double), hipMemcpyDeviceToDevice, st));
             if (mp > m) hipLaunchKernelGGL(set_diagonal_kernel, dim3((unsigned)((mp - m + kBlock - 1) / kBlock)), dim3(kBlock), 0, st, Sinv.p, mp, m, mp, 1.0);
-            enqueue_gj_invert(Sinv.p, mp, true);
+            if (plan.s_factor) enqueue_ldl_factor(Sinv.p, mp, ldlP, ldlPanels);
+            else enqueue_gj_invert(Sinv.p, mp, true);
             Sinv_ones.alloc((size_t)2 * mp);
             hipLaunchKernelGGL(fill_kernel, dim3((unsigned)((m + kBlock - 1) / kBlock)), dim3(kBlock), 0, st, Sinv_ones.p + mp, m, 1.0);
-            launch_ginv_matvec<double>(st, m, m, mp, Sinv.p, Sinv_ones.p + mp, Sinv_ones.p);
+            if (plan.s_factor) {
+                ldlWork.alloc((size_t)3 * mp);
+                apply_ldl(st, m, mp, Sinv.p, ldlP.p, ldlWork.p, Sinv_ones.p + mp, Sinv_ones.p);
+            } else launch_ginv_matvec<double>(st, m, m, mp, Sinv.p, Sinv_ones.p + mp, Sinv_ones.p);
         } else {
             e_sch_done->record(st);
             HIPCHK(hipStreamWaitEvent(stream2, e_sch_done->e, 0));
@@ -2062,7 +2102,10 @@
         };
         bool finished = false;
         if (direct) {
-            auto apply_Sinv = [&](const double* w, double* u) { launch_ginv_matvec<double>(stream, m, m, mp, Sinv.p, w, u); };
+            auto apply_Sinv = [&](const double* w, double* u) {
+                if (plan.s_factor) apply_ldl(stream, m, mp, Sinv.p, ldlP.p, ldlWork.p, w, u);
+                else launch_ginv_matvec<double>(stream, m, m, mp, Sinv.p, w, u);
+            };
             const int max_passes = std::min(o.max_iters, 6);
             double rr_prev = -1.;
             while (it < max_passes && !converged && !breakdown) {
@@ -2610,6 +2653,36 @@
         if (!have_S) throw Error(SHM_ERR_STATE, "no explicit Schur complement for this problem (several slabs, more than 16384 rows, or n = 2^k where the plan applies S through the grid: n > 512, or the estimate of plan_explicit_S without SHM_DUAL_DENSE_S_ALWAYS)");
         HIPCHK(hipMemcpy2DAsync(out, (size_t)m * sizeof(double), Sdense.p, (size_t)mp * sizeof(double), (size_t)m * sizeof(double), (size_t)m, hipMemcpyDeviceToHost, stream2));
         HIPCHK(hipStreamSynchronize(stream2));
+    }
+
+    void spd_solve(const double* S, int32_t m_, const double* rhs, int32_t form, double* u, int32_t* flag) override {
+        if (cfg.world != 1) throw Error(SHM_ERR_INVALID, "spd_solve is a single-process test entry point");
+        if (m_ < 1 || m_ > 4096 || (form != 0 && form != 1)) throw Error(SHM_ERR_INVALID, "spd_solve: m in [1, 4096], form 0 (factor) or 1 (invert)");
+        const int mp_ = (m_ + kGJ - 1) / kGJ * kGJ;
+        if (form == 0 && !ldl_applies(mp_ / kGJ)) throw Error(SHM_ERR_INVALID, "spd_solve: the factorisation serves fewer than 64 pivot blocks");
+        HIPCHK(hipSetDevice(cfg.device));
+        hipStream_t st = stream2;
+        DevArray<double> M, Pd, panels, vecs;
+        M.alloc((size_t)mp_ * mp_);
+        vecs.alloc((size_t)5 * mp_);
+        HIPCHK(hipMemsetAsync(M.p, 0, (size_t)mp_ * mp_ * sizeof(double), st));
+        HIPCHK(hipMemsetAsync(vecs.p, 0, (size_t)5 * mp_ * sizeof(double), st));
+        HIPCHK(hipMemcpy2DAsync(M.p, (size_t)mp_ * sizeof(double), S, (size_t)m_ * sizeof(double), (size_t)m_ * sizeof(double), (size_t)m_, hipMemcpyHostToDevice, st));
+        HIPCHK(hipMemcpyAsync(vecs.p, rhs, (size_t)m_ * sizeof(double), hipMemcpyHostToDevice, st));
+        if (mp_ > m_) hipLaunchKernelGGL(set_diagonal_kernel, dim3((unsigned)((mp_ - m_ + kBlock - 1) / kBlock)), dim3(kBlock), 0, st, M.p, mp_, m_, mp_, 1.0);
+        if (form == 0) {
+            enqueue_ldl_factor(M.p, mp_, Pd, panels);
+            apply_ldl(st, m_, mp_, M.p, Pd.p, vecs.p + 2 * (size_t)mp_, vecs.p, vecs.p + mp_);
+        } else {
+            enqueue_gj_invert(M.p, mp_, true);
+            launch_ginv_matvec<double>(st, m_, m_, mp_, M.p, vecs.p, vecs.p + mp_);
+        }
+        HIPCHK(hipGetLastError());
+        int f = 0;
+        HIPCHK(hipMemcpyAsync(&f, gjFlag.p, sizeof(int), hipMemcpyDeviceToHost, st));
+        HIPCHK(hipMemcpyAsync(u, vecs.p + mp_, (size_t)m_ * sizeof(double), hipMemcpyDeviceToHost, st));
+        HIPCHK(hipStreamSynchronize(st));
+        *flag = f;
     }
 
     void apply_projector(double* v) override {
diff --git a/signed-heat-3d_amd/grid_abi.py b/signed-heat-3d_amd/grid_abi.py
--- a/signed-heat-3d_amd/grid_abi.py
+++ b/signed-heat-3d_amd/grid_abi.py
@@ -13,7 +13,7 @@
 
 ABI_SYMBOLS = ["shm_grid_owned_planes", "shm_grid_create", "shm_grid_destroy", "shm_grid_last_error", "shm_grid_abi_version", "shm_grid_set_problem",
                "shm_grid_solve", "shm_grid_get_phi", "shm_grid_compute_distance", "shm_grid_run_conv", "shm_grid_run_conv_arith", "shm_grid_run_divergence",
-               "shm_grid_get_field", "shm_grid_get_field_planes", "shm_grid_apply_laplacian", "shm_grid_set_phi", "shm_grid_get_constraints", "shm_grid_get_schur", "shm_grid_apply_projector", "shm_grid_apply_preconditioner", "shm_grid_isosurface", "shm_grid_isosurface_ex", "shm_grid_get_isosurface",
+               "shm_grid_get_field", "shm_grid_get_field_planes", "shm_grid_apply_laplacian", "shm_grid_set_phi", "shm_grid_get_constraints", "shm_grid_get_schur", "shm_grid_spd_solve", "shm_grid_apply_projector", "shm_grid_apply_preconditioner", "shm_grid_isosurface", "shm_grid_isosurface_ex", "shm_grid_get_isosurface",
                "shm_grid_isosurface_indexed", "shm_grid_get_isosurface_indexed", "shm_grid_get_isosurface_indexed_device",
                "shm_grid_label_mesh_device", "shm_grid_isosurface_components", "shm_grid_get_isosurface_components", "shm_grid_isosurface_keep_components",
                "shm_grid_sample", "shm_grid_sample_device", "shm_grid_raycast", "shm_grid_raycast_device",
@@ -141,6 +141,8 @@
     lib.shm_grid_set_phi.argtypes = [C.c_void_p, C.c_void_p]
     lib.shm_grid_get_constraints.argtypes = [C.c_void_p, C.c_void_p, C.c_void_p, C.POINTER(C.c_int32)]
     lib.shm_grid_get_schur.argtypes = [C.c_void_p, C.c_void_p, C.POINTER(C.c_int32)]
+    if hasattr(lib, "shm_grid_spd_solve"):
+        lib.shm_grid_spd_solve.argtypes = [C.c_void_p, C.c_void_p, C.c_int32, C.c_void_p, C.c_int32, C.c_void_p, C.POINTER(C.c_int32)]
     lib.shm_grid_apply_projector.argtypes = [C.c_void_p, C.c_void_p]
     lib.shm_grid_apply_preconditioner.argtypes = [C.c_void_p, C.c_void_p, C.c_void_p]
     lib.shm_grid_isosurface.argtypes = [C.c_void_p, C.c_double, C.POINTER(C.c_int64), C.POINTER(C.c_int64)]
@@ -357,6 +359,17 @@
         assert mm.value == m
         return out
 
+    def spd_solve(self, S, rhs, form="factor"):
+        S = np.ascontiguousarray(S, dtype=np.float64)
+        rhs = np.ascontiguousarray(rhs, dtype=np.float64).reshape(-1)
+        m = S.shape[0]
+        if S.shape != (m, m) or rhs.size != m:
+            raise ValueError("spd_solve: S must be m x m and rhs hold m values")
+        u = np.empty(m, dtype=np.float64)
+        flag = C.c_int32(0)
+        self._chk(self._lib.shm_grid_spd_solve(self._h, S.ctypes.data, m, rhs.ctypes.data, {"factor": 0, "invert": 1}[form], u.ctypes.data, C.byref(flag)))
+        return u, flag.value
+
     def apply_projector(self, v):
         v = _f64(v).reshape(-1).copy()
         self._chk(self._lib.shm_grid_apply_projector(self._h, v.ctypes.data))
```

New measurement: 713.3 million, median of 6. +1.7%, better.
